# marbl/MashMap

Measured on AMD Instinct MI355X. Metric: query Gbp/s sketch+L1/L2 map (pi=85, s=5000), higher is better.
Workload: dtype u64

## Files before the change

mashmap_amd/csrc/mm_api.hip:

```cpp
#include <chrono>
#include "mm_internal.h"
#include <algorithm>
#include <cstring>
#include <thread>
#include "../host/mm_stats.hpp"
#include "../host/pack2bit.hpp"

static thread_local std::string g_createErr;

static const char* kKernelNames[MM_K_COUNT] = {
  "k_pack2bit", "k_sketch_fast", "k_sketch_hard", "k_seed_lookup", "k_sort_points",
  "k_l1_sweep", "k_l2_sweep", "k_ref_hash", "k_l2_locate", "k_winnow_tiles", "k_l2_select"};

mm_env mm_read_env() {
  mm_env v;
  v.debug = getenv("MM_DEBUG") != nullptr;
  v.timing = getenv("MASHMAP_HIP_TIMING") != nullptr;
  v.sketchStats = getenv("MM_SKETCH_STATS") != nullptr;
  v.l1Literal = getenv("MM_L1_LITERAL") != nullptr;
  if (const char* e = getenv("MM_L2_PRE_LIMIT")) { const int x = atoi(e); if (x >= 0 && x < 4000) v.l2PreLimit = x; }
  if (const char* e = getenv("MM_L2_STREAM_MIB")) { const double x = atof(e); if (x > 0) v.l2StreamMiB = x; }
  v.winnowGsk = getenv("MM_WINNOW_GSK") != nullptr;
  if (const char* e = getenv("MM_SEED_TAGS")) v.seedTags = atoi(e) != 0;
  if (const char* e = getenv("MASHMAP_HIP_RCCL")) v.rcclPath = e;
  v.noRccl = getenv("MASHMAP_HIP_NO_RCCL") != nullptr;
  v.requireRccl = getenv("MASHMAP_HIP_REQUIRE_RCCL") != nullptr;
  return v;
}

std::vector<DevBuf*> mm_ctx::allBufs() {
  DeviceIndex& I = idx;
  return {&I.evKey, &I.evAux, &I.evHash, &I.contigOff, &I.opKey, &I.opAux, &I.opHash, &I.blockOff, &I.evBlock, &I.contigBlock, &I.contigLen, &I.refGroup,
          &I.htSlots, &I.htTags, &I.filter, &I.ptKeys, &I.keys, &I.keyOff, &I.keyFreq, &dMinHits, &dCutoffs, &dAscii, &dAsciiNext, &dReadSrcOff, &dReadPackOff, &dReadLen, &dReadGroup, &dReadSelf, &dReadHasN,
          &dBases2, &dNmask, &dFrags, &dSkHash, &dSkPos, &dSkStrand, &dSkCount, &dHardList, &dCounters, &dSketchSpill, &dSketchTabs, &dQHash, &dQStrand,
          &dStats, &dPtOff, &dPts, &dPtKept, &dPtIds, &dWinFreq, &dWinExt, &dWinHeap, &dWinKeys, &dWinVals, &dWinOffH, &dWinOffT, &dWinCntH, &dWinCntT, &dL1, &dL1b, &dL1Cursors, &dL1Off, &dL1Regions, &dL2, &dL2Info, &dL2Cnt, &dL2Off, &dL2Ops, &dScanTmp, &dL2Tmp, &dL2Wide, &dL2Exact, &dL2Cells,
          &dListB, &dListC, &dBigList, &dMidList, &dL2Sort[0], &dL2Sort[1], &dL2Sort[2], &dL2Sort[3], &dL2Order, &dL2OrderPos, &dL2InitCells, &dL2InitState, &dL2First, &dL2Num, &dAccept, &dMinIsz, &dSelCnt, &dSelOff, &dSelHeap, &dFragTab, &dMappings, &dCommCounts, &dGathered};
}

extern "C" {

int mm_abi_version(void) { return MM_ABI_VERSION; }
const char* mm_kernel_name(int which) { return (which >= 0 && which < MM_K_COUNT) ? kKernelNames[which] : "?"; }

const char* mm_last_error(const mm_ctx* ctx) { return ctx ? ctx->err.c_str() : g_createErr.c_str(); }

int mm_create(mm_ctx** out, int device, const mm_params* p) {
  if (!out || !p) { g_createErr = "mm_create: null argument"; return MM_ERR_ARG; }
  *out = nullptr;
  if (p->kmerSize < 1 || p->kmerSize > 64 || p->sketchSize < 1 || p->segLength < p->kmerSize) {
    g_createErr = "mm_create: unsupported parameters (need 1 <= kmerSize <= 64, sketchSize >= 1, segLength >= kmerSize)";
    return MM_ERR_ARG;
  }
  if (mm_check_params(p, g_createErr) != MM_OK) return MM_ERR_ARG;
  int ndev = 0;
  hipError_t e = hipGetDeviceCount(&ndev);
  if (e != hipSuccess || ndev <= 0 || device < 0 || device >= ndev) {
    g_createErr = std::string("mm_create: no usable HIP device (") + (e == hipSuccess ? "index out of range" : hipGetErrorString(e)) + ")";
    return MM_ERR_DEVICE;
  }
  if ((e = hipSetDevice(device)) != hipSuccess) { g_createErr = hipGetErrorString(e); return MM_ERR_DEVICE; }
  hipDeviceProp_t prop;
  if ((e = hipGetDeviceProperties(&prop, device)) != hipSuccess) { g_createErr = hipGetErrorString(e); return MM_ERR_DEVICE; }
  if (std::string(prop.gcnArchName).find("gfx950") == std::string::npos) {
    g_createErr = std::string("mm_create: kernels are built for gfx950 only, device is ") + prop.gcnArchName;
    return MM_ERR_DEVICE;
  }
  mm_ctx* c = new mm_ctx();
  c->device = device; c->P = *p; c->env = mm_read_env();
  if ((e = hipStreamCreateWithFlags(&c->stream, hipStreamNonBlocking)) != hipSuccess ||
      (e = hipEventCreate(&c->evA)) != hipSuccess || (e = hipEventCreate(&c->evB)) != hipSuccess) {
    g_createErr = hipGetErrorString(e); delete c; return MM_ERR_DEVICE;
  }
  *out = c;
  return MM_OK;
}

void mm_destroy(mm_ctx* c) {
  if (!c) return;
  (void)hipSetDevice(c->device);
  (void)hipStreamSynchronize(c->stream);
  if (c->gatherThread.joinable()) c->gatherThread.join();
  mm_comm_release(c);
  if (c->commStream) (void)hipStreamDestroy(c->commStream);
  if (c->copyStream) { (void)hipStreamSynchronize(c->copyStream); (void)hipStreamDestroy(c->copyStream); }
  if (c->copyDone) (void)hipEventDestroy(c->copyDone);
  for (DevBuf* b : c->allBufs()) b->release();
  c->dGatherSrc.release();
  for (auto& p : c->parked)
    for (DevBuf* b : {&p.dReadSrcOff, &p.dReadPackOff, &p.dReadLen, &p.dReadGroup, &p.dReadSelf, &p.dReadHasN, &p.dBases2, &p.dNmask, &p.dFrags}) b->release();
  if (c->hPass) (void)hipHostFree(c->hPass);
  for (auto& pr : c->evPool) { (void)hipEventDestroy(pr.first); (void)hipEventDestroy(pr.second); }
  if (c->evA) (void)hipEventDestroy(c->evA);
  if (c->evB) (void)hipEventDestroy(c->evB);
  if (c->stream) (void)hipStreamDestroy(c->stream);
  delete c;
}

int mm_synchronize(mm_ctx* c) { MM_HIP(c, hipStreamSynchronize(c->stream)); return MM_OK; }
void* mm_stream(const mm_ctx* c) { return (void*)c->stream; }

int mm_set_option(mm_ctx* c, int option, int value) {
  if (option == MM_OPT_KEEP_POINTS) { c->keepPoints = value != 0; c->keepFiltered = value == 2; c->ptsCap = 0; return MM_OK; }
  if (option == MM_OPT_KEEP_FULL_INDEX) { c->keepFullIndex = value != 0; return MM_OK; }
  if (option == MM_OPT_RESERVE_FRAGMENTS) { c->reserveFrags = value > 0 ? (size_t)value : 0; return MM_OK; }
  c->err = "mm_set_option: unknown option"; return MM_ERR_ARG;
}

int mm_profile_enable(mm_ctx* c, int on) { c->profile = on != 0; return MM_OK; }
int mm_profile_read(mm_ctx* c, double* ms, uint64_t* launches, int reset) {
  if (!c->evPending.empty()) { MM_HIP(c, hipSetDevice(c->device)); MM_HIP(c, hipStreamSynchronize(c->stream)); mm_profile_collect(c); }
  for (int i = 0; i < MM_K_COUNT; i++) { if (ms) ms[i] = c->kMs[i]; if (launches) launches[i] = c->kLaunches[i]; }
  if (reset) for (int i = 0; i < MM_K_COUNT; i++) { c->kMs[i] = 0; c->kLaunches[i] = 0; }
  return MM_OK;
}

int mm_index_upload(mm_ctx* c, const mm_minmer* minmers, size_t nMinmers, const uint64_t* keys, const uint64_t* offsets,
                    size_t nKeys, const mm_interval_point* points, size_t nPoints, const uint64_t* freqSeeds, size_t nFreq,
                    const int32_t* contigLen, const int32_t* refGroup, size_t nContigs) {
  if ((nMinmers && !minmers) || (nKeys && (!keys || !offsets)) || (nPoints && !points) || (nFreq && !freqSeeds) || !contigLen || !nContigs) {
    c->err = "mm_index_upload: null argument"; return MM_ERR_ARG;
  }
  MM_HIP(c, hipSetDevice(c->device));
  c->mirrorMinmers = c->mirrorMap = false;
  c->hMinmers.assign(minmers, minmers + nMinmers);
  c->hKeys.assign(keys, keys + nKeys);
  c->hOffsets.assign(offsets, offsets + nKeys + (nKeys ? 1 : 0));
  if (!nKeys) c->hOffsets.assign(1, 0);
  c->hPoints.assign(points, points + nPoints);
  c->hFreq.assign(freqSeeds, freqSeeds + nFreq);
  std::sort(c->hFreq.begin(), c->hFreq.end());
  if (c->hOffsets.back() != nPoints) { c->err = "mm_index_upload: offsets[nKeys] != nPoints"; return MM_ERR_ARG; }
  c->mapped = false;
  return mm_build_device_index(c, contigLen, refGroup, nContigs);
}

int mm_set_tables(mm_ctx* c, const int32_t* minHits, size_t nMinHits, const int32_t* cutoffs, size_t nCutoffs) {
  if (!minHits || nMinHits < (size_t)c->P.sketchSize + 1 || !cutoffs || nCutoffs < 2) {
    c->err = "mm_set_tables: need sketchSize+1 minHits entries and the sketchCutoffs table"; return MM_ERR_ARG;
  }
  MM_HIP(c, hipSetDevice(c->device));
  MM_HIP(c, c->dMinHits.ensure(nMinHits * 4));
  MM_HIP(c, c->dCutoffs.ensure(nCutoffs * 4));
  MM_HIP(c, hipMemcpyAsync(c->dMinHits.p, minHits, nMinHits * 4, hipMemcpyHostToDevice, c->stream));
  MM_HIP(c, hipMemcpyAsync(c->dCutoffs.p, cutoffs, nCutoffs * 4, hipMemcpyHostToDevice, c->stream));
  MM_HIP(c, hipStreamSynchronize(c->stream));
  c->nMinHits = nMinHits; c->nCutoffs = nCutoffs;
  return MM_OK;
}

int mm_set_tables_default(mm_ctx* c, float pi) {
  const int s = c->P.sketchSize, k = c->P.kmerSize;
  std::vector<int32_t> mh = mmhost::minHitsTable(s, k, pi);
  std::vector<int> cut = mmhost::sketchCutoffs(s, k, mmhost::fixed::ANIDiff, mmhost::fixed::ANIDiffConf, (c->P.flags & MM_FLAG_HG_FILTER) != 0);
  std::vector<int32_t> cut32(cut.begin(), cut.end());
  int rc = mm_set_tables(c, mh.data(), mh.size(), cut32.data(), cut32.size());
  if (rc != MM_OK) return rc;
  std::vector<uint8_t> accept; std::vector<int16_t> minIsz;
  mmhost::replayTables(s, k, pi, mmhost::fixed::ANIDiff, true, std::max(1u, std::thread::hardware_concurrency()), accept, minIsz);
  return mm_set_replay_tables(c, accept.data(), minIsz.data(), (size_t)s + 1);
}

float mm_stat_j2md(float j, int k) { return mmhost::Stat::j2md(j, k); }
float mm_stat_md2j(float d, int k) { return mmhost::Stat::md2j(d, k); }
float mm_stat_md_lower_bound(float d, int s, int k, float ci) { return mmhost::Stat::md_lower_bound(d, s, k, ci); }
int mm_stat_min_hits_relaxed(int s, int k, float pi) { return mmhost::Stat::estimateMinimumHitsRelaxed(s, k, pi, mmhost::fixed::confidence_interval); }
int64_t mm_stat_recommended_sketch_size(int k, float pi, int64_t segLength, uint64_t referenceSize) {
  return mmhost::Stat::recommendedSketchSize(mmhost::fixed::pval_cutoff, mmhost::fixed::confidence_interval, k, 4, pi, segLength, referenceSize);
}
int mm_stat_replay_tables(int sketchSize, int k, float percentageIdentity, float ANIDiff, int keepLowPctId, uint8_t* accept, int16_t* minIsz) {
  if (sketchSize < 1 || !accept || !minIsz) return MM_ERR_ARG;
  std::vector<uint8_t> a; std::vector<int16_t> m;
  mmhost::replayTables(sketchSize, k, percentageIdentity, ANIDiff, keepLowPctId != 0, std::max(1u, std::thread::hardware_concurrency()), a, m);
  std::memcpy(accept, a.data(), a.size()); std::memcpy(minIsz, m.data(), m.size() * 2);
  return MM_OK;
}
int mm_stat_sketch_cutoffs(int sketchSize, int k, int hgFilter, int32_t* out, size_t cap) {
  std::vector<int> cut = mmhost::sketchCutoffs(sketchSize, k, mmhost::fixed::ANIDiff, mmhost::fixed::ANIDiffConf, hgFilter != 0);
  size_t n = std::min(cap, cut.size());
  for (size_t i = 0; i < n; i++) out[i] = cut[i];
  return (int)cut.size();
}

static inline void cut_read(mm_ctx* c, std::vector<DFrag>& dfr, size_t r, int32_t len, int64_t pk, int32_t& maxLen, bool& anyLong) {
  const int k = c->P.kmerSize, L = c->P.segLength;
  const bool split = !(c->P.flags & MM_FLAG_NO_SPLIT);
  if (len < k) return;
  if (!split || len <= L) {
    if (len > L) anyLong = true;
    c->hFrags.push_back(mm_fragment{(int32_t)r, 0, len, 0});
    dfr.push_back(DFrag{pk, len, (int32_t)r});
    maxLen = std::max(maxLen, len);
    return;
  }
  const int nfull = len / L;
  for (int i = 0; i < nfull; i++) {
    c->hFrags.push_back(mm_fragment{(int32_t)r, i * L, L, 0});
    dfr.push_back(DFrag{pk + (int64_t)i * L, L, (int32_t)r});
  }
  if (nfull >= 1 && len % L != 0) {
    c->hFrags.push_back(mm_fragment{(int32_t)r, len - L, L, 0});
    dfr.push_back(DFrag{pk + (int64_t)(len - L), L, (int32_t)r});
  }
  maxLen = std::max(maxLen, L);
}

static int finish_upload(mm_ctx* c, size_t nReads, int64_t pk, const std::vector<int64_t>& srcOff, const std::vector<int64_t>& packOff, const std::vector<int32_t>& rlen,
                         const std::vector<int32_t>& grp, const std::vector<int32_t>& self, const std::vector<uint32_t>* hasN32, const std::vector<DFrag>& dfr, bool packOnDevice) {
  MM_HIP(c, hipMemcpyAsync(c->dReadSrcOff.p, srcOff.data(), (nReads + 1) * 8, hipMemcpyHostToDevice, c->stream));
  MM_HIP(c, hipMemcpyAsync(c->dReadPackOff.p, packOff.data(), (nReads + 1) * 8, hipMemcpyHostToDevice, c->stream));
  if (nReads) {
    MM_HIP(c, hipMemcpyAsync(c->dReadLen.p, rlen.data(), nReads * 4, hipMemcpyHostToDevice, c->stream));
    MM_HIP(c, hipMemcpyAsync(c->dReadGroup.p, grp.data(), nReads * 4, hipMemcpyHostToDevice, c->stream));
    MM_HIP(c, hipMemcpyAsync(c->dReadSelf.p, self.data(), nReads * 4, hipMemcpyHostToDevice, c->stream));
  }
  if (hasN32) MM_HIP(c, hipMemcpyAsync(c->dReadHasN.p, hasN32->data(), nReads * 4 + 4, hipMemcpyHostToDevice, c->stream));
  else MM_HIP(c, hipMemsetAsync(c->dReadHasN.p, 0, nReads * 4 + 4, c->stream));
  MM_HIP(c, hipMemsetAsync((char*)c->dBases2.p + pk / 4, 0, 64, c->stream));
  MM_HIP(c, hipMemsetAsync((char*)c->dNmask.p + pk / 8, 0, 64, c->stream));
  if (!dfr.empty()) MM_HIP(c, hipMemcpyAsync(c->dFrags.p, dfr.data(), dfr.size() * sizeof(DFrag), hipMemcpyHostToDevice, c->stream));
  if (packOnDevice) { const int rc = mm_launch_pack(c); if (rc != MM_OK) return rc; }
  MM_HIP(c, hipStreamSynchronize(c->stream));
  return MM_OK;
}

static int ensure_read_buffers(mm_ctx* c, size_t nReads, int64_t pk, size_t nFrags) {
  if (c->reserveFrags > nFrags) {
    const int64_t pkR = (int64_t)c->reserveFrags * (int64_t)c->P.segLength; pk = pkR > pk ? pkR + pkR / 64 : pk;
    nReads = std::max(nReads, c->reserveFrags); nFrags = c->reserveFrags;
  }
  MM_HIP(c, c->dReadSrcOff.ensure((nReads + 1) * 8)); MM_HIP(c, c->dReadPackOff.ensure((nReads + 1) * 8));
  MM_HIP(c, c->dReadLen.ensure(nReads * 4 + 4)); MM_HIP(c, c->dReadGroup.ensure(nReads * 4 + 4)); MM_HIP(c, c->dReadSelf.ensure(nReads * 4 + 4));
  MM_HIP(c, c->dReadHasN.ensure(nReads * 4 + 4));
  MM_HIP(c, c->dBases2.ensure((size_t)pk / 4 + 64)); MM_HIP(c, c->dNmask.ensure((size_t)pk / 8 + 64));
  MM_HIP(c, c->dFrags.ensure(nFrags * sizeof(DFrag) + 16));
  return MM_OK;
}

static int upload_reads_ascii(mm_ctx* c, const void* ascii, bool onDevice, const int64_t* readOffsets, size_t nReads, const int32_t* readRefGroup,
                              const int32_t* readSelfSeqId, int32_t seqCounterBase) {
  if (!readOffsets) { c->err = "mm_reads_upload: null argument"; return MM_ERR_ARG; }
  std::lock_guard<std::mutex> prefetchLock(c->prefetchMu);
  MM_HIP(c, hipSetDevice(c->device));
  std::vector<int64_t> srcOff(nReads + 1), packOff(nReads + 1);
  std::vector<int32_t> rlen(nReads);
  c->hFrags.clear();
  std::vector<DFrag> dfr;
  dfr.reserve(c->hFrags.capacity() ? c->hFrags.capacity() : nReads * 2 + 16);
  int64_t pk = 0; int32_t maxLen = 0; bool anyLong = false;
  for (size_t r = 0; r < nReads; r++) {
    const int64_t len64 = readOffsets[r + 1] - readOffsets[r];
    if (len64 < 0 || len64 > 0x7fffffff) { c->err = "mm_reads_upload: read length out of range (offset_t is int32, base_types.hpp:21)"; return MM_ERR_ARG; }
    srcOff[r] = readOffsets[r]; packOff[r] = pk; rlen[r] = (int32_t)len64;
    cut_read(c, dfr, r, (int32_t)len64, pk, maxLen, anyLong);
    pk += (len64 + 31) / 32 * 32;
  }
  srcOff[nReads] = readOffsets[nReads]; packOff[nReads] = pk;
  c->nReads = nReads; c->nFrags = dfr.size(); c->nPackedBases = (size_t)pk; c->seqCounterBase = seqCounterBase; c->maxFragLen = maxLen;
  c->sketched = false; c->mapped = false; c->fragTabStale = true; c->gathered = false;
  c->windowed = anyLong;
  const size_t srcBase = (size_t)readOffsets[0];
  const size_t nSrc = (size_t)(readOffsets[nReads] - readOffsets[0]);
  if (nSrc && !ascii) { c->err = "mm_reads_upload: null argument"; return MM_ERR_ARG; }
  for (size_t r = 0; r <= nReads; r++) srcOff[r] -= (int64_t)srcBase;
  const bool prefetched = c->prefetchValid && !onDevice && nSrc && c->prefetchPtr == (const void*)((const char*)ascii + srcBase) && c->prefetchBytes == nSrc;
  c->prefetchValid = false;
  c->staged.clear(); c->stagedBytes = 0;
  if (prefetched) { std::swap(c->dAscii, c->dAsciiNext); MM_HIP(c, hipStreamWaitEvent(c->stream, c->copyDone, 0)); }
  else MM_HIP(c, c->dAscii.ensure(nSrc + 64));
  { const int rc = ensure_read_buffers(c, nReads, pk, dfr.size()); if (rc != MM_OK) return rc; }
  if (nSrc && !prefetched) MM_HIP(c, hipMemcpyAsync(c->dAscii.p, (const char*)ascii + srcBase, nSrc, onDevice ? hipMemcpyDeviceToDevice : hipMemcpyHostToDevice, c->stream));
  std::vector<int32_t> grp(nReads, -1), self(nReads, -1);
  if (readRefGroup) grp.assign(readRefGroup, readRefGroup + nReads);
  if (readSelfSeqId) self.assign(readSelfSeqId, readSelfSeqId + nReads);
  return finish_upload(c, nReads, pk, srcOff, packOff, rlen, grp, self, nullptr, dfr, true);
}

static int upload_packed_parts(mm_ctx* c, const mm_packed_part* parts, size_t nParts, int32_t seqCounterBase) {
  if (nParts && !parts) { c->err = "mm_reads_upload_packed: null argument"; return MM_ERR_ARG; }
  std::lock_guard<std::mutex> prefetchLock(c->prefetchMu);
  MM_HIP(c, hipSetDevice(c->device));
  size_t nReads = 0;
  for (size_t p = 0; p < nParts; p++) {
    if (parts[p].nReads && !parts[p].readLengths) { c->err = "mm_reads_upload_packed: null argument"; return MM_ERR_ARG; }
    nReads += parts[p].nReads;
  }
  if (nReads > 0x7fffffff) { c->err = "mm_reads_upload_packed: more than 2^31 reads in one batch"; return MM_ERR_ARG; }
  std::vector<int64_t> srcOff(nReads + 1, 0), packOff(nReads + 1);
  std::vector<int32_t> rlen(nReads), grp(nReads, -1), self(nReads, -1);
  std::vector<uint32_t> hasN32(nReads + 1, 0u);
  std::vector<int64_t> partBase(nParts + 1, 0);
  c->hFrags.clear();
  std::vector<DFrag> dfr;
  dfr.reserve(c->hFrags.capacity() ? c->hFrags.capacity() : nReads * 2 + 16);
  int64_t pk = 0; int32_t maxLen = 0; bool anyLong = false;
  size_t r = 0;
  for (size_t p = 0; p < nParts; p++) {
    const mm_packed_part& P = parts[p];
    partBase[p] = pk;
    int64_t at = 0;
    for (size_t i = 0; i < P.nReads; i++, r++) {
      const int64_t len64 = (int64_t)P.readLengths[i];
      if (len64 < 0) { c->err = "mm_reads_upload_packed: negative read length"; return MM_ERR_ARG; }
      if (P.readStarts) {
        const int64_t want = P.readStarts[i] - P.readStarts[0];
        if (want < at || (want & 31)) { c->err = "mm_reads_upload_packed: readStarts must be ascending multiples of 32 that leave room for every read"; return MM_ERR_ARG; }
        at = want;
      }
      packOff[r] = pk + at; rlen[r] = (int32_t)len64;
      if (P.readRefGroup) grp[r] = P.readRefGroup[i];
      if (P.readSelfSeqId) self[r] = P.readSelfSeqId[i];
      if (P.readHasN) hasN32[r] = P.readHasN[i] ? 1u : 0u;
      else if (len64) {
        if (!P.nmask) { c->err = "mm_reads_upload_packed: null argument"; return MM_ERR_ARG; }
        const uint32_t* w = P.nmask + at / 32; const size_t nw = ((size_t)len64 + 31) / 32;
        uint32_t any = 0; for (size_t j = 0; j < nw; j++) any |= w[j];
        hasN32[r] = any ? 1u : 0u;
      }
      cut_read(c, dfr, r, (int32_t)len64, pk + at, maxLen, anyLong);
      at += (len64 + 31) / 32 * 32;
    }
    if (at && (!P.bases2 || !P.nmask)) { c->err = "mm_reads_upload_packed: null argument"; return MM_ERR_ARG; }
    pk += at;
  }
  partBase[nParts] = pk; packOff[nReads] = pk;
  c->nReads = nReads; c->nFrags = dfr.size(); c->nPackedBases = (size_t)pk; c->seqCounterBase = seqCounterBase; c->maxFragLen = maxLen;
  c->sketched = false; c->mapped = false; c->fragTabStale = true; c->gathered = false;
  c->windowed = anyLong;
  c->prefetchValid = false;
  { const int rc = ensure_read_buffers(c, nReads, pk, dfr.size()); if (rc != MM_OK) return rc; }
  bool waited = false;
  std::vector<char> used(c->staged.size(), 0);
  for (size_t p = 0; p < nParts; p++) {
    const int64_t n = partBase[p + 1] - partBase[p];
    if (!n) continue;
    char* dB = (char*)c->dBases2.p + partBase[p] / 4; char* dM = (char*)c->dNmask.p + partBase[p] / 8;
    size_t hit = c->staged.size();
    for (size_t q = 0; q < c->staged.size(); q++)
      if (!used[q] && c->staged[q].b2 == (const void*)parts[p].bases2 && c->staged[q].nm == (const void*)parts[p].nmask && c->staged[q].nPacked == (size_t)n) { hit = q; break; }
    if (hit < c->staged.size()) {
      if (!waited) { MM_HIP(c, hipStreamWaitEvent(c->stream, c->copyDone, 0)); waited = true; }
      used[hit] = 1;
      const char* src = (const char*)c->dAsciiNext.p + c->staged[hit].off;
      MM_HIP(c, hipMemcpyAsync(dB, src, (size_t)n / 4, hipMemcpyDeviceToDevice, c->stream));
      MM_HIP(c, hipMemcpyAsync(dM, src + (size_t)n / 4, (size_t)n / 8, hipMemcpyDeviceToDevice, c->stream));
    } else {
      MM_HIP(c, hipMemcpyAsync(dB, parts[p].bases2, (size_t)n / 4, hipMemcpyHostToDevice, c->stream));
      MM_HIP(c, hipMemcpyAsync(dM, parts[p].nmask, (size_t)n / 8, hipMemcpyHostToDevice, c->stream));
    }
  }
  const int rc = finish_upload(c, nReads, pk, srcOff, packOff, rlen, grp, self, &hasN32, dfr, false);
  std::vector<mm_ctx::StagedPart> left;
  for (size_t q = 0; q < c->staged.size(); q++) if (!used[q]) left.push_back(c->staged[q]);
  c->staged.swap(left);
  return rc;
}

int mm_reads_upload(mm_ctx* c, const char* bases, const int64_t* readOffsets, size_t nReads, const int32_t* g, const int32_t* s, int32_t base) {
  return upload_reads_ascii(c, bases, false, readOffsets, nReads, g, s, base);
}
int mm_reads_upload_device(mm_ctx* c, const void* dBases, size_t nBases, const int64_t* readOffsets, size_t nReads, const int32_t* g,
                           const int32_t* s, int32_t base) {
  (void)nBases;
  return upload_reads_ascii(c, dBases, true, readOffsets, nReads, g, s, base);
}
int mm_reads_upload_packed(mm_ctx* c, const uint32_t* bases2, const uint32_t* nmask, const uint8_t* readHasN, const int32_t* readLengths, const int64_t* readStarts,
                           size_t nReads, const int32_t* g, const int32_t* s, int32_t base) {
  static const int32_t none = 0;
  mm_packed_part P{bases2, nmask, readHasN, readLengths ? readLengths : &none, nReads ? readStarts : nullptr, nReads, g, s};
  return upload_packed_parts(c, &P, 1, base);
}
int mm_reads_upload_packed_parts(mm_ctx* c, const mm_packed_part* parts, size_t nParts, int32_t base) { return upload_packed_parts(c, parts, nParts, base); }
size_t mm_pack_read(const char* ascii, size_t len, uint32_t* bases2, uint32_t* nmask) { return mmhost::pack2bit(ascii, len, bases2, nmask); }
size_t mm_pack_read_portable(const char* ascii, size_t len, uint32_t* bases2, uint32_t* nmask) { return mmhost::pack2bit_scalar(ascii, len, bases2, nmask); }

int mm_reads_packed_download(mm_ctx* c, uint32_t* bases2, uint32_t* nmask, uint32_t* readHasN, size_t* nPackedBases) {
  if (nPackedBases) *nPackedBases = c->nPackedBases;
  MM_HIP(c, hipSetDevice(c->device));
  if (bases2 && c->nPackedBases) MM_HIP(c, hipMemcpyAsync(bases2, c->dBases2.p, c->nPackedBases / 4, hipMemcpyDeviceToHost, c->stream));
  if (nmask && c->nPackedBases) MM_HIP(c, hipMemcpyAsync(nmask, c->dNmask.p, c->nPackedBases / 8, hipMemcpyDeviceToHost, c->stream));
  if (readHasN && c->nReads) MM_HIP(c, hipMemcpyAsync(readHasN, c->dReadHasN.p, c->nReads * 4, hipMemcpyDeviceToHost, c->stream));
  MM_HIP(c, hipStreamSynchronize(c->stream));
  return MM_OK;
}

static int prefetch_streams(mm_ctx* c) {
  MM_HIP(c, hipSetDevice(c->device));
  if (!c->copyStream) MM_HIP(c, hipStreamCreateWithFlags(&c->copyStream, hipStreamNonBlocking));
  if (!c->copyDone) MM_HIP(c, hipEventCreateWithFlags(&c->copyDone, hipEventDisableTiming));
  return MM_OK;
}

int mm_reads_prefetch(mm_ctx* c, const char* bases, size_t nBytes) {
  std::lock_guard<std::mutex> prefetchLock(c->prefetchMu);
  c->prefetchValid = false;
  if (!bases || !nBytes) return MM_OK;
  { const int rc = prefetch_streams(c); if (rc != MM_OK) return rc; }
  c->staged.clear(); c->stagedBytes = 0;
  MM_HIP(c, c->dAsciiNext.ensure(nBytes + 64));
  MM_HIP(c, hipMemcpyAsync(c->dAsciiNext.p, bases, nBytes, hipMemcpyHostToDevice, c->copyStream));
  MM_HIP(c, hipEventRecord(c->copyDone, c->copyStream));
  c->prefetchPtr = bases; c->prefetchPtr2 = nullptr; c->prefetchBytes = nBytes; c->prefetchPacked = false; c->prefetchValid = true;
  return MM_OK;
}

static int stage_packed(mm_ctx* c, const uint32_t* bases2, const uint32_t* nmask, size_t nPackedBases, size_t reservePackedBases, int* stagedOut = nullptr) {
  if (stagedOut) *stagedOut = 0;
  if (nPackedBases % 32) { c->err = "mm_reads_prefetch_packed: the packed length of a batch is a multiple of 32 bases"; return MM_ERR_ARG; }
  { const int rc = prefetch_streams(c); if (rc != MM_OK) return rc; }
  c->prefetchValid = false;
  const size_t bytes = nPackedBases / 4 + nPackedBases / 8;
  if (c->staged.empty()) {
    const size_t want = std::max(bytes, reservePackedBases / 4 + reservePackedBases / 8) + 64;
    MM_HIP(c, c->dAsciiNext.ensure(want));
    c->stagedBytes = 0;
  }
  auto fits = [&](size_t off) {
    if (off + bytes + 64 > c->dAsciiNext.bytes) return false;
    for (const auto& q : c->staged) { const size_t qb = q.nPacked / 4 + q.nPacked / 8; if (off < q.off + qb && q.off < off + bytes) return false; }
    return true;
  };
  if (!fits(c->stagedBytes)) {
    if (!fits(0)) return MM_OK;
    c->stagedBytes = 0;
  }
  char* dst = (char*)c->dAsciiNext.p + c->stagedBytes;
  MM_HIP(c, hipMemcpyAsync(dst, bases2, nPackedBases / 4, hipMemcpyHostToDevice, c->copyStream));
  MM_HIP(c, hipMemcpyAsync(dst + nPackedBases / 4, nmask, nPackedBases / 8, hipMemcpyHostToDevice, c->copyStream));
  MM_HIP(c, hipEventRecord(c->copyDone, c->copyStream));
  c->staged.push_back(mm_ctx::StagedPart{bases2, nmask, nPackedBases, c->stagedBytes});
  c->stagedBytes += bytes;
  if (stagedOut) *stagedOut = 1;
  return MM_OK;
}

int mm_reads_prefetch_packed(mm_ctx* c, const uint32_t* bases2, const uint32_t* nmask, size_t nPackedBases) {
  std::lock_guard<std::mutex> prefetchLock(c->prefetchMu);
  c->prefetchValid = false;
  c->staged.clear(); c->stagedBytes = 0;
  if (!bases2 || !nmask || !nPackedBases) return MM_OK;
  return stage_packed(c, bases2, nmask, nPackedBases, nPackedBases);
}

int mm_reads_prefetch_packed_append(mm_ctx* c, const uint32_t* bases2, const uint32_t* nmask, size_t nPackedBases, size_t reservePackedBases, int* staged) {
  std::lock_guard<std::mutex> prefetchLock(c->prefetchMu);
  if (staged) *staged = 0;
  if (!bases2 || !nmask || !nPackedBases) return MM_OK;
  return stage_packed(c, bases2, nmask, nPackedBases, reservePackedBases, staged);
}

int mm_reads_prefetch_reserve(mm_ctx* c, size_t reservePackedBases) {
  std::lock_guard<std::mutex> prefetchLock(c->prefetchMu);
  if (!c->staged.empty() || c->prefetchValid) return MM_OK;
  { const int rc = prefetch_streams(c); if (rc != MM_OK) return rc; }
  MM_HIP(c, c->dAsciiNext.ensure(reservePackedBases / 4 + reservePackedBases / 8 + 64));
  return MM_OK;
}

int mm_reads_prefetch_drop(mm_ctx* c) {
  std::lock_guard<std::mutex> prefetchLock(c->prefetchMu);
  c->prefetchValid = false;
  c->staged.clear(); c->stagedBytes = 0;
  return MM_OK;
}

void* mm_host_alloc(size_t bytes) {
  void* p = nullptr;
  if (hipHostMalloc(&p, bytes ? bytes : 1, hipHostMallocDefault) != hipSuccess) return nullptr;
  return p;
}
void mm_host_free(void* p) { if (p) (void)hipHostFree(p); }

int mm_reads_exchange(mm_ctx* c, int slot) {
  if (slot < 0 || slot >= MM_BATCH_SLOTS) { c->err = "mm_reads_exchange: slot out of range"; return MM_ERR_ARG; }
  std::lock_guard<std::mutex> prefetchLock(c->prefetchMu);
  MM_HIP(c, hipSetDevice(c->device));
  MM_HIP(c, hipStreamSynchronize(c->stream));
  mm_ctx::ParkedReads& p = c->parked[slot];
  std::swap(c->nReads, p.nReads); std::swap(c->nFrags, p.nFrags); std::swap(c->nPackedBases, p.nPackedBases);
  std::swap(c->seqCounterBase, p.seqCounterBase); std::swap(c->maxFragLen, p.maxFragLen); std::swap(c->windowed, p.windowed);
  std::swap(c->dReadSrcOff, p.dReadSrcOff); std::swap(c->dReadPackOff, p.dReadPackOff); std::swap(c->dReadLen, p.dReadLen);
  std::swap(c->dReadGroup, p.dReadGroup); std::swap(c->dReadSelf, p.dReadSelf); std::swap(c->dReadHasN, p.dReadHasN);
  std::swap(c->dBases2, p.dBases2); std::swap(c->dNmask, p.dNmask); std::swap(c->dFrags, p.dFrags);
  c->hFrags.swap(p.hFrags);
  c->sketched = false; c->mapped = false; c->fragTabStale = true; c->gathered = false;
  return MM_OK;
}

size_t mm_num_fragments(const mm_ctx* c) { return c->nFrags; }
int mm_fragments_download(mm_ctx* c, mm_fragment* out) {
  if (c->nFrags) std::memcpy(out, c->hFrags.data(), c->nFrags * sizeof(mm_fragment));
  return MM_OK;
}

int mm_sketch_fragments(mm_ctx* c) {
  MM_HIP(c, hipSetDevice(c->device));
  int rc = mm_launch_sketch(c);
  if (rc != MM_OK) return rc;
  MM_HIP(c, hipStreamSynchronize(c->stream));
  if (c->profile) mm_profile_collect(c);
  c->sketched = true;
  return MM_OK;
}

int mm_sketch_download(mm_ctx* c, mm_minmer* out, uint32_t* counts) {
  if (!c->sketched) { c->err = "mm_sketch_download: no sketches resident"; return MM_ERR_STATE; }
  MM_HIP(c, hipSetDevice(c->device));
  const size_t nF = c->nFrags, s = (size_t)c->P.sketchSize;
  std::vector<uint64_t> h(nF * s); std::vector<int2> p(nF * s); std::vector<int8_t> st(nF * s); std::vector<uint32_t> cnt(nF);
  if (nF) {
    MM_HIP(c, hipMemcpyAsync(h.data(), c->dSkHash.p, nF * s * 8, hipMemcpyDeviceToHost, c->stream));
    MM_HIP(c, hipMemcpyAsync(p.data(), c->dSkPos.p, nF * s * 8, hipMemcpyDeviceToHost, c->stream));
    MM_HIP(c, hipMemcpyAsync(st.data(), c->dSkStrand.p, nF * s, hipMemcpyDeviceToHost, c->stream));
    MM_HIP(c, hipMemcpyAsync(cnt.data(), c->dSkCount.p, nF * 4, hipMemcpyDeviceToHost, c->stream));
    MM_HIP(c, hipStreamSynchronize(c->stream));
  }
  for (size_t f = 0; f < nF; f++) {
    if (counts) counts[f] = cnt[f];
    if (!out) continue;
    for (uint32_t r = 0; r < cnt[f]; r++) {
      const size_t o = f * s + r;
      out[o] = mm_minmer{h[o], p[o].x, p[o].y, c->hFrags[f].readId + c->seqCounterBase, (int16_t)st[o], 0};
    }
  }
  return MM_OK;
}

int mm_map_fragments(mm_ctx* c) {
  if (!c->idx.ready) { c->err = "mm_map_fragments: no index resident (mm_index_upload / mm_index_build first)"; return MM_ERR_STATE; }
  if (!c->nMinHits) { c->err = "mm_map_fragments: mm_set_tables first"; return MM_ERR_STATE; }
  MM_HIP(c, hipSetDevice(c->device));
  const auto t0 = std::chrono::steady_clock::now();
  const double a0 = g_mmAllocSeconds;
  int rc = mm_launch_sketch(c);
  if (rc != MM_OK) return rc;
  c->sketched = true;
  const auto t1 = std::chrono::steady_clock::now();
  rc = mm_launch_map(c);
  if (rc != MM_OK) return rc;
  if (!c->lastSteady) { MM_HIP(c, hipStreamSynchronize(c->stream)); c->nSyncs++; }
  if (c->env.timing && !c->lastSteady) {
    auto sec = [](std::chrono::steady_clock::time_point a, std::chrono::steady_clock::time_point b) { return std::chrono::duration<double>(b - a).count(); };
    fprintf(stderr, "[mashmap_hip::timing] sized pass (%zu fragments, %llu host waits): sketch launch %.4f s, lookup .. selection %.4f s, of both in hipMalloc / hipFree %.4f s\n",
            c->nFrags, (unsigned long long)c->nSyncs, sec(t0, t1), sec(t1, std::chrono::steady_clock::now()), g_mmAllocSeconds - a0);
  }
  if (c->profile) mm_profile_collect(c);
  c->mapped = true;
  c->nPasses++; if (c->lastSteady) c->nSteadyPasses++;
  return MM_OK;
}

int mm_pass_totals(const mm_ctx* c, uint64_t* passes, uint64_t* steadyPasses, uint64_t* redonePasses) {
  if (passes) *passes = c->nPasses;
  if (steadyPasses) *steadyPasses = c->nSteadyPasses;
  if (redonePasses) *redonePasses = c->nRedone;
  return MM_OK;
}

int mm_pass_redo_cause(const mm_ctx* c, uint64_t* cause) {
  if (cause) *cause = c->redoCause;
  return MM_OK;
}

int mm_pass_stats(const mm_ctx* c, uint64_t* hostSyncs, int* steady, uint64_t* counts) {
  if (!c->mapped) return MM_ERR_STATE;
  if (hostSyncs) *hostSyncs = c->nSyncs;
  if (steady) *steady = c->lastSteady ? 1 : 0;
  if (counts) { counts[0] = c->nL1; counts[1] = c->nL2; counts[2] = c->lastBig; counts[3] = c->lastOps; counts[4] = c->lastHard; }
  return MM_OK;
}

int mm_result_counts(const mm_ctx* c, size_t* nL1, size_t* nL2) {
  if (!c->mapped) return MM_ERR_STATE;
  if (nL1) *nL1 = c->nL1;
  if (nL2) *nL2 = c->nL2;
  return MM_OK;
}

int mm_results_device(const mm_ctx* c, const mm_l2_locus** dL2, size_t* nL2) {
  if (!c->mapped) return MM_ERR_STATE;
  if (dL2) *dL2 = c->dL2.as<mm_l2_locus>();
  if (nL2) *nL2 = c->nL2;
  return MM_OK;
}

int mm_results_copy_device(mm_ctx* c, mm_l2_locus* dDst, size_t cap, size_t* n) {
  if (!c->mapped) { c->err = "mm_results_copy_device: nothing mapped"; return MM_ERR_STATE; }
  if (n) *n = c->nL2;
  if (c->nL2 > cap) { c->err = "mm_results_copy_device: destination too small"; return MM_ERR_ARG; }
  if (c->nL2) MM_HIP(c, hipMemcpyAsync(dDst, c->dL2.p, c->nL2 * sizeof(mm_l2_locus), hipMemcpyDeviceToDevice, c->stream));
  MM_HIP(c, hipStreamSynchronize(c->stream));
  return MM_OK;
}

int mm_index_sizes(const mm_ctx* c, size_t* nMinmers, size_t* nKeys, size_t* nPoints, size_t* nFreq, int32_t* freqThreshold) {
  if (!c->idx.ready) return MM_ERR_STATE;
  if (nMinmers) *nMinmers = c->idx.nRec;
  if (nKeys) *nKeys = c->idx.nKeys;
  if (nPoints) *nPoints = c->idx.nPoints;
  if (nFreq) *nFreq = c->hFreq.size();
  if (freqThreshold) *freqThreshold = c->freqThreshold;
  return MM_OK;
}

int mm_index_layout_get(const mm_ctx* c, mm_index_layout* o) {
  if (!c->idx.ready || !o) return MM_ERR_STATE;
  const DeviceIndex& I = c->idx;
  o->seedTableSlots = I.htCap; o->seedTableBytes = (uint64_t)I.htCap * 16;
  o->tagged = I.tagged ? 1 : 0; o->pad_ = 0;
  o->tagBytes = I.tagged ? (uint64_t)I.htCap : 0;
  o->filterBytes = I.filterMask ? (I.filterMask + 1) * 8 : 0;
  o->events = 2 * (uint64_t)I.nRec; o->openRecords = I.nOpen;
  return MM_OK;
}

int mm_index_download(mm_ctx* c, mm_minmer* minmers, uint64_t* keys, uint64_t* offsets, mm_interval_point* points, uint64_t* freqSeeds) {
  if (!c->idx.ready) { c->err = "mm_index_download: no index resident"; return MM_ERR_STATE; }
  if (c->idx.keys.bytes == 0 && c->idx.nKeys) { c->err = "mm_index_download: this context holds a replica (mm_index_replicate); ask the context the index was built on"; return MM_ERR_STATE; }
  MM_HIP(c, hipSetDevice(c->device));
  if (minmers) { const int rc = mm_mirror_minmers(c); if (rc != MM_OK) return rc; }
  if (keys || offsets || points) { const int rc = mm_mirror_map(c); if (rc != MM_OK) return rc; }
  if (minmers && !c->hMinmers.empty()) std::memcpy(minmers, c->hMinmers.data(), c->hMinmers.size() * sizeof(mm_minmer));
  if (keys && !c->hKeys.empty()) std::memcpy(keys, c->hKeys.data(), c->hKeys.size() * 8);
  if (offsets) std::memcpy(offsets, c->hOffsets.data(), c->hOffsets.size() * 8);
  if (points && !c->hPoints.empty()) std::memcpy(points, c->hPoints.data(), c->hPoints.size() * sizeof(mm_interval_point));
  if (freqSeeds && !c->hFreq.empty()) std::memcpy(freqSeeds, c->hFreq.data(), c->hFreq.size() * 8);
  return MM_OK;
}

}
```

mashmap_amd/csrc/mm_internal.h:

```cpp
#pragma once
#include <chrono>
#include <hip/hip_runtime.h>
#include <stdint.h>
#include <mutex>
#include <string>
#include <thread>
#include <utility>
#include <vector>
#include "../../include/mashmap_hip.h"

#define MM_WAVE 64

inline double g_mmAllocSeconds = 0.0;
struct DevBuf {
  void* p = nullptr;
  size_t bytes = 0;
  hipError_t ensure(size_t need) {
    if (need <= bytes) return hipSuccess;
    const auto t0 = std::chrono::steady_clock::now();
    void* q = nullptr;
    size_t cap = need + need / 8 + 256;
    hipError_t e = hipMalloc(&q, cap);
    if (e != hipSuccess) {
      (void)hipGetLastError();
      if (p) { (void)hipFree(p); p = nullptr; bytes = 0; }
      e = hipMalloc(&q, cap);
      if (e != hipSuccess) { (void)hipGetLastError(); cap = need + 256; e = hipMalloc(&q, cap); }
    } else if (p) {
      (void)hipFree(p);
    }
    if (e == hipSuccess) { p = q; bytes = cap; }
    g_mmAllocSeconds += std::chrono::duration<double>(std::chrono::steady_clock::now() - t0).count();
    return e;
  }
  void release() { if (p) (void)hipFree(p); p = nullptr; bytes = 0; }
  template <class T> T* as() const { return reinterpret_cast<T*>(p); }
};

struct DFrag {
  int64_t base;
  int32_t len;
  int32_t readId;
};


#define MM_OPEN_BLOCK_SHIFT 10

struct DeviceIndex {
  size_t nRec = 0, nKeys = 0, nPoints = 0, nContigs = 0, htCap = 0, nOpen = 0;
  DevBuf evKey;
  DevBuf evAux;
  DevBuf evHash;
  DevBuf contigOff;
  DevBuf opKey, opAux, opHash;
  DevBuf blockOff;
  DevBuf evBlock;
  DevBuf contigBlock;
  DevBuf contigLen;
  DevBuf refGroup;
  DevBuf htSlots;
  DevBuf filter; uint64_t filterMask = 0;
  DevBuf htTags; bool tagged = false;
  DevBuf ptKeys;
  DevBuf keys, keyOff, keyFreq;
  bool ready = false;
};

enum : int {
  MM_CW_SKETCH        = 0,
  MM_CW_SKETCH_END    = 8,
  MM_CW_PASS          = 8,
  MM_CW_PASS_END      = 16,
  MM_CW_SORT_LENS     = 16,
  MM_CW_SORT_LENS_END = 18,
  MM_CW_INDEX_BUILD   = 16,
  MM_CW_INDEX_FLATTEN = 20,
  MM_CW_INDEX_END     = 24,
  MM_CW_MID_LEN       = 24,
  MM_CW_SKETCH_PHASES = 24,
  MM_CW_SKETCH_PHASES_END = 32,
  MM_CW_MAP           = 32,
  MM_CW_MAP_END       = 40,
  MM_CW_HARD_COPY     = 48,
  MM_CW_WORDS         = 64
};
#define MM_COUNTER_BYTES ((size_t)MM_CW_WORDS * 8)

enum : int {
  MM_PC_POINT_CURSOR   = 0,
  MM_PC_L2_EXACT_LEN   = 0,
  MM_PC_POINT_OVERFLOW = 1,
  MM_PC_L1_CAND        = 2,
  MM_PC_L1_OVERFLOW    = 3,
  MM_PC_L2_LOCI        = 4,
  MM_PC_L2_OVERFLOW    = 5,
  MM_PC_L2_FLAGS       = 6,
  MM_PC_BIG_LEN        = 7,
  MM_PC_L2_WIDE_LEN    = 7,
  MM_PC_READ           = MM_CW_PASS_END - MM_CW_PASS,
  MM_PC_MID_LEN        = MM_CW_MID_LEN - MM_CW_PASS
};
constexpr unsigned long long MM_OVERFLOWED = 1ull;
constexpr unsigned long long MM_L2F_SLOTS  = 1ull;
constexpr unsigned long long MM_L2F_STREAM = 4ull;
constexpr unsigned long long MM_L2F_OPS    = 8ull;
constexpr unsigned long long MM_L2F_LIST   = 16ull;
constexpr unsigned long long MM_L2F_CANDS  = 32ull;
__host__ __device__ inline bool mm_pass_incomplete(const unsigned long long* pc) {
  return (pc[MM_PC_POINT_OVERFLOW] | pc[MM_PC_L1_OVERFLOW] | pc[MM_PC_L2_OVERFLOW] | pc[MM_PC_L2_FLAGS]) != 0;
}
enum : int {
  MM_MC_MAPPINGS = 0,
  MM_MC_OVERFLOW = 1,
  MM_MC_L2_OPS   = 2
};
inline uint64_t mm_redo_cause(const unsigned long long* pc, const unsigned long long* mc) {
  const unsigned long long f = pc[MM_PC_L2_FLAGS];
  uint64_t cause = 0;
  if (pc[MM_PC_POINT_OVERFLOW]) cause |= MM_REDO_POINTS;
  if (pc[MM_PC_L1_OVERFLOW]) cause |= MM_REDO_L1;
  if (pc[MM_PC_L2_OVERFLOW]) cause |= MM_REDO_L2_LOCI;
  if (f & MM_L2F_SLOTS) cause |= MM_REDO_L2_SLOTS;
  if (f & MM_L2F_STREAM) cause |= MM_REDO_L2_STREAM;
  if (f & MM_L2F_OPS) cause |= MM_REDO_L2_OPS;
  if (f & MM_L2F_LIST) cause |= MM_REDO_L2_LIST;
  if (f & MM_L2F_CANDS) cause |= MM_REDO_L2_CANDS;
  if (mc[MM_MC_OVERFLOW]) cause |= MM_REDO_MAPPINGS;
  return cause;
}
enum : int {
  MM_SL_BLOCK   = 0,
  MM_SL_GLOBAL  = 1,
  MM_SL_LITERAL = 2,
  MM_SL_END     = 4
};
enum : int {
  MM_IX_BUILD_UNSTABLE = 0,
  MM_IX_BUILD_NFREQ    = 1,
  MM_IX_BUILD_CURSOR   = 2,
  MM_IX_BUILD_THRESHOLD = 3,
  MM_IX_FLAT_BAD_REC   = 1,
  MM_IX_FLAT_MAX_LEN   = 2,
  MM_IX_FLAT_TABLE     = 3
};
static_assert(MM_CW_SKETCH_END <= MM_CW_PASS && MM_CW_PASS_END <= MM_CW_SORT_LENS && MM_CW_SORT_LENS_END <= MM_CW_MID_LEN, "mapping pass: parts overlap");
static_assert(MM_CW_SORT_LENS * 2 + MM_SL_END <= MM_CW_SORT_LENS_END * 2, "the 32-bit list lengths outgrow their words");
static_assert(MM_CW_MID_LEN < MM_CW_MAP && MM_CW_MAP + MM_MC_L2_OPS < MM_CW_MAP_END && MM_CW_MAP_END <= MM_CW_HARD_COPY && MM_CW_HARD_COPY < MM_CW_WORDS, "mapping pass: parts overlap");
static_assert(MM_CW_INDEX_BUILD + 4 == MM_CW_INDEX_FLATTEN && MM_CW_INDEX_FLATTEN + 4 == MM_CW_INDEX_END && MM_CW_SKETCH_END <= MM_CW_INDEX_BUILD, "index build: parts overlap");
static_assert(MM_CW_SKETCH_PHASES >= MM_CW_INDEX_END && MM_CW_SKETCH_PHASES_END <= MM_CW_MAP, "the sketch statistics must stay clear of the words that outlive the sketch launcher");
static_assert(MM_PC_POINT_CURSOR == MM_PC_L2_EXACT_LEN && MM_PC_BIG_LEN == MM_PC_L2_WIDE_LEN, "the words shared by the L1 stage and the L2 sweep");
static_assert(MM_CW_PASS + MM_PC_MID_LEN == MM_CW_SKETCH_PHASES, "k_lookup_mid's list length shares its word with the sketch statistics");
static_assert(MM_PC_L2_LOCI + 1 == MM_PC_L2_OVERFLOW && MM_PC_L2_OVERFLOW + 1 == MM_PC_L2_FLAGS && MM_PC_L2_FLAGS < MM_PC_READ, "the L2 words are reset as one range");
static_assert(MM_PC_L1_CAND + 1 == MM_PC_L1_OVERFLOW, "the L1 cursor and its flag are read back as one range");

struct mm_env {
  bool debug = false;
  bool timing = false;
  bool sketchStats = false;
  bool l1Literal = false;
  int l2PreLimit = 4000;
  double l2StreamMiB = 0;
  bool winnowGsk = false;
  int seedTags = -1;
  std::string rcclPath;
  bool noRccl = false;
  bool requireRccl = false;
};
mm_env mm_read_env();

struct mm_ctx {
  int device = 0;
  hipStream_t stream = nullptr;
  mm_params P{};
  mm_env env;
  std::string err;

  std::vector<mm_minmer> hMinmers;
  std::vector<mm_minmer> hMinmersAll;
  bool keepFullIndex = false;
  std::vector<uint64_t> hKeys, hOffsets, hFreq;
  std::vector<mm_interval_point> hPoints;
  bool mirrorMinmers = false, mirrorMap = false;
  int32_t freqThreshold = 0x7fffffff;

  DeviceIndex idx;
  DevBuf dMinHits, dCutoffs; size_t nMinHits = 0, nCutoffs = 0;

  size_t nReads = 0, nFrags = 0, nPackedBases = 0;
  int32_t seqCounterBase = 0, maxFragLen = 0;
  DevBuf dAscii, dReadSrcOff, dReadPackOff, dReadLen, dReadGroup, dReadSelf, dReadHasN;
  DevBuf dAsciiNext; hipStream_t copyStream = nullptr; hipEvent_t copyDone = nullptr;
  const void* prefetchPtr = nullptr; const void* prefetchPtr2 = nullptr; size_t prefetchBytes = 0; bool prefetchValid = false, prefetchPacked = false;
  struct StagedPart { const void* b2; const void* nm; size_t nPacked; size_t off; };
  std::vector<StagedPart> staged; size_t stagedBytes = 0;
  std::mutex prefetchMu;
  DevBuf dBases2, dNmask, dFrags;
  std::vector<mm_fragment> hFrags;
  struct ParkedReads {
    size_t nReads = 0, nFrags = 0, nPackedBases = 0; int32_t seqCounterBase = 0, maxFragLen = 0; bool windowed = false;
    DevBuf dReadSrcOff, dReadPackOff, dReadLen, dReadGroup, dReadSelf, dReadHasN, dBases2, dNmask, dFrags;
    std::vector<mm_fragment> hFrags;
  };
  ParkedReads parked[MM_BATCH_SLOTS];

  DevBuf dSkHash, dSkPos, dSkStrand, dSkCount;
  DevBuf dHardList, dCounters, dSketchSpill;
  DevBuf dSketchTabs; int sketchTabsK = 0;
  DevBuf dQHash, dQStrand;
  DevBuf dStats;
  DevBuf dPtOff, dPts; size_t ptsCap = 0;
  DevBuf dPtKept;
  bool windowed = false;
  DevBuf dPtIds, dWinFreq, dWinExt, dWinHeap, dWinKeys, dWinVals, dWinOffH, dWinOffT, dWinCntH, dWinCntT;
  DevBuf dL1, dL1b, dL1Cursors; size_t l1Cap = 0, nL1 = 0;
  DevBuf dL1Off;
  DevBuf dL1Regions;
  DevBuf dL2; size_t l2Cap = 0, nL2 = 0;
  DevBuf dL2First, dL2Num;
  DevBuf dAccept, dMinIsz; bool haveReplayTables = false;
  DevBuf dSelCnt, dSelOff, dSelHeap, dFragTab, dMappings; size_t nMappings = 0; bool fragTabStale = true;
  void* comm = nullptr; int commRank = 0, commWorld = 0; bool commCopy = false;
  DevBuf dCommCounts, dGathered; std::vector<size_t> gatherCounts, gatherDisp; size_t nGathered = 0; bool gathered = false;
  DevBuf dGatherSrc; hipStream_t commStream = nullptr; std::thread gatherThread; int gatherRc = 0; std::string gatherErr;
  std::vector<DevBuf*> allBufs();
  DevBuf dL2Info, dL2Cnt, dL2Off, dL2Ops, dScanTmp, dL2Tmp, dL2Wide, dL2Exact, dL2Cells, dListB, dListC, dBigList, dMidList;
  DevBuf dL2InitCells, dL2InitState;
  DevBuf dL2Sort[4], dL2Order, dL2OrderPos;
  bool sketched = false, mapped = false;
  bool steadyOk = false, lastSteady = false; size_t prevBig = 0, candCap = 0, l2Chunks = 1, sizedFrags = 0; int prevLocap = 0, steadyFails = 0;
  unsigned long long* hPass = nullptr;
  size_t lastHard = 0;
  size_t prevMid = 0, lastMid = 0; bool midKnown = false;
  size_t lastOps = 0, lastBig = 0;
  size_t nSyncs = 0;
  uint64_t nPasses = 0, nSteadyPasses = 0, nRedone = 0;
  uint64_t redoCause = 0;
  bool keepFiltered = false;
  bool keepPoints = false;
  size_t reserveFrags = 0;

  bool profile = false;
  double kMs[MM_K_COUNT] = {0};
  uint64_t kLaunches[MM_K_COUNT] = {0};
  hipEvent_t evA = nullptr, evB = nullptr;
  std::vector<std::pair<hipEvent_t, hipEvent_t>> evPool; size_t evUsed = 0;
  std::vector<std::pair<int, size_t>> evPending;
};

#define MM_HIP(ctx, call)                                                                        \
  do {                                                                                           \
    hipError_t e__ = (call);                                                                     \
    if (e__ != hipSuccess) {                                                                     \
      (ctx)->err = std::string(#call) + ": " + hipGetErrorString(e__);                           \
      return MM_ERR_DEVICE;                                                                      \
    }                                                                                            \
  } while (0)
#define MM_SYNC(c) do { MM_HIP(c, hipStreamSynchronize((c)->stream)); (c)->nSyncs++; } while (0)

struct KernelTimer {
  mm_ctx* c; int which; size_t idx = 0; bool on = false;
  KernelTimer(mm_ctx* c_, int w) : c(c_), which(w) {
    if (!c->profile) return;
    if (c->evUsed == c->evPool.size()) {
      if (c->evPool.size() >= 8192) return;
      hipEvent_t a = nullptr, b = nullptr;
      if (hipEventCreate(&a) != hipSuccess || hipEventCreate(&b) != hipSuccess) { if (a) (void)hipEventDestroy(a); c->profile = false; return; }
      c->evPool.emplace_back(a, b);
    }
    idx = c->evUsed++;
    on = hipEventRecord(c->evPool[idx].first, c->stream) == hipSuccess;
  }
  ~KernelTimer() {
    if (!on) return;
    if (hipEventRecord(c->evPool[idx].second, c->stream) == hipSuccess) c->evPending.emplace_back(which, idx);
  }
};
inline void mm_profile_collect(mm_ctx* c) {
  for (const auto& pr : c->evPending) {
    float ms = 0;
    if (hipEventElapsedTime(&ms, c->evPool[pr.second].first, c->evPool[pr.second].second) == hipSuccess) { c->kMs[pr.first] += ms; c->kLaunches[pr.first] += 1; }
  }
  c->evPending.clear(); c->evUsed = 0;
}

inline size_t mm_frag_cap(const mm_ctx* c, size_t nF) { return nF > c->reserveFrags ? nF : c->reserveFrags; }
inline size_t mm_scaled(const mm_ctx* c, size_t count, size_t bytesPer) {
  const size_t nF = c->nFrags ? c->nFrags : 1;
  if (c->reserveFrags <= nF) return count;
  size_t scaled = (size_t)((double)count * (double)c->reserveFrags / (double)nF) + 1;
  size_t freeB = 0, totalB = 0;
  if (hipMemGetInfo(&freeB, &totalB) != hipSuccess) { (void)hipGetLastError(); return count; }
  const size_t most = freeB / 8 / (bytesPer ? bytesPer : 1);
  if (scaled > most) scaled = most > count ? most : count;
  return scaled;
}

int mm_check_params(const mm_params* p, std::string& err);
int mm_launch_pack(mm_ctx* c);
int mm_launch_pack_raw(mm_ctx* c, const uint8_t* dAscii, const int64_t* dSrcOff, const int64_t* dPackOff, const int32_t* dLen, int nReads,
                       int64_t nChunks, uint32_t* dB, uint32_t* dM, uint32_t* dHasN);
int mm_launch_sketch(mm_ctx* c);
int mm_launch_sketch_global(mm_ctx* c);
#define MM_LDS_MAX_SKETCH 8190
#define MM_WINNOW_LDS_SKETCH 4096
#define MM_MAX_SKETCH 65535
int mm_launch_map(mm_ctx* c);
#define MM_PASS_REDO 1
int mm_launch_select(mm_ctx* c, bool steady = false);
void mm_comm_release(mm_ctx* c);
int mm_launch_l2(mm_ctx* c, unsigned long long* cnt, bool steady = false);
int mm_build_device_index(mm_ctx* c, const int32_t* contigLen, const int32_t* refGroup, size_t nContigs);
int mm_flatten_device_index(mm_ctx* c, const mm_minmer* dRec, size_t n, size_t nk, size_t np, const int32_t* contigLen, const int32_t* refGroup, size_t nContigs);
int mm_finalize_index_device(mm_ctx* c, const std::vector<std::pair<const mm_minmer*, size_t>>& parts, float kmerPctThreshold, const int32_t* contigLen,
                             const int32_t* refGroup, size_t nContigs);
int mm_mirror_minmers(mm_ctx* c);
int mm_mirror_map(mm_ctx* c);
int mm_scan_i32_to_i64(mm_ctx* c, int64_t n, const int32_t* dIn, int64_t* dOut, int64_t* total);
int mm_scan_i32_to_i64_dev(mm_ctx* c, int64_t n, const int32_t* dIn, int64_t* dOut, const int64_t** dTotal);
int mm_order_desc(mm_ctx* c, const int32_t* dKey, int c0, int n, int shift, int32_t* dOrder);
int mm_order_pairs(mm_ctx* c, int n, unsigned bits, int32_t* dOrder);
```

mashmap_amd/csrc/mm_sketch.hip:

```cpp
#include "mm_internal.h"
#include "mm_device.h"
#include <cmath>
#include <cstdio>
#include <cstdlib>

__global__ void k_pack2bit(const uint8_t* __restrict__ ascii, const int64_t* __restrict__ srcOff,
                           const int64_t* __restrict__ packOff, const int32_t* __restrict__ readLen, int nReads,
                           int64_t nChunks, uint32_t* __restrict__ bases2, uint32_t* __restrict__ nmask,
                           uint32_t* __restrict__ readHasN) {
  for (int64_t c = (int64_t)blockIdx.x * blockDim.x + threadIdx.x; c < nChunks; c += (int64_t)gridDim.x * blockDim.x) {
    const int64_t b0 = c * 32;
    int lo = 0, hi = nReads;
    while (hi - lo > 1) { int mid = (lo + hi) >> 1; if (packOff[mid] <= b0) lo = mid; else hi = mid; }
    const int r = lo;
    const int64_t local = b0 - packOff[r];
    const int len = readLen[r];
    uint32_t wlo = 0, whi = 0, nm = 0;
    if (local < len) {
      const uint8_t* src = ascii + srcOff[r] + local;
      const int cnt = (len - local) < 32 ? (int)(len - local) : 32;
      for (int i = 0; i < cnt; i++) {
        const uint32_t ch = src[i] & 0xDFu;
        const bool ok = (ch == 'A') | (ch == 'C') | (ch == 'G') | (ch == 'T');
        const uint32_t code = ok ? (((ch >> 1) ^ (ch >> 2)) & 3u) : 0u;
        if (i < 16) wlo |= code << (2 * i); else whi |= code << (2 * (i - 16));
        nm |= (ok ? 0u : 1u) << i;
      }
    }
    bases2[2 * c] = wlo; bases2[2 * c + 1] = whi;
    nmask[c] = nm;
    if (nm) atomicOr(&readHasN[r], 1u);
  }
}

#define MM_SK_PAD 64
#define MM_SK_PADH 256
#define MM_SK_DUPCAP 256
#define MM_SK_GUARD 4
enum : int { MM_TC_KEYS = 0 , MM_TC_OVERFLOW = 1 , MM_TC_OCCUPIED = 2 , MM_TC_DUPS = 3  };
struct SkTable {
  uint64_t* key; int32_t* first; int32_t* last; int32_t* sum;
  uint32_t* counters;
  uint64_t* occW; uint32_t* occP;
  uint32_t nSlots, maxLoad, M; int sh;

  __device__ __forceinline__ void set_cut(uint64_t T, uint32_t HT) {
    sh = (T == MM_HASH_MAX) ? 0 : __clzll((long long)T);
    const uint64_t t32 = ((T << sh) >> 32) + 1ull;
    M = (uint32_t)((float)HT * 4294967296.0f / (float)t32 * 0.99999f);
  }
  __device__ __forceinline__ uint32_t home(uint64_t h) const { return __umulhi((uint32_t)((h << sh) >> 32), M); }

  __device__ __forceinline__ void insert(uint64_t h, int pos, int st) {
    uint32_t slot = home(h);
    for (uint32_t probes = 1;; probes++) {
      if ((probes & 15u) == 0 && ((volatile uint32_t*)counters)[MM_TC_OVERFLOW]) return;
      const unsigned long long prev = atomicCAS((unsigned long long*)&key[slot], (unsigned long long)MM_HASH_MAX,
                                                (unsigned long long)h);
      if (prev == MM_HASH_MAX) {
        if (atomicAdd(&counters[MM_TC_KEYS], 1u) >= maxLoad) atomicOr(&counters[MM_TC_OVERFLOW], 1u);
      }
      if (prev == MM_HASH_MAX || prev == h) {
        atomicMin(&first[slot], pos); atomicMax(&last[slot], pos); atomicAdd(&sum[slot], st);
        return;
      }
      if (++slot >= nSlots) { atomicOr(&counters[MM_TC_OVERFLOW], 1u); return; }
    }
  }
};

__host__ __device__ static inline int sketch_fast_queue_total(int QC, int nWaves, int HT) { const int a = QC * nWaves, b = HT * 5 / 8 + 1; return ((a > b ? a : b) + 3) & ~3; }

template <int K>
__device__ __forceinline__ uint64_t mm_window_or(uint64_t x) {
  constexpr int P = K >= 32 ? 32 : K >= 16 ? 16 : K >= 8 ? 8 : K >= 4 ? 4 : K >= 2 ? 2 : 1;
  uint64_t w = x;
#pragma unroll
  for (int d = 1; d < P; d <<= 1) w |= w >> d;
  return w | (w >> (K - P));
}

#define MM_SK_HINT_OVERFLOW 0xFFFFFFFFu
template <int K, bool SPILL>
__device__ __forceinline__ void
mm_sketch_hard(unsigned char* smem, const int f, const uint4* __restrict__ gTabs, const uint32_t* __restrict__ bases2, const uint32_t* __restrict__ nmask,
               const DFrag* __restrict__ frags, const uint32_t* __restrict__ readHasN, int s, int wantFast, int HT, int PAD, int32_t* __restrict__ spill,
               const bool stream ,
               uint64_t* __restrict__ skHash, int2* __restrict__ skPos, int8_t* __restrict__ skStrand, uint32_t* __restrict__ skCount) {
  const DFrag fr = frags[f];
  const int len = fr.len;
  const int n = len - K + 1;
  const int tid = threadIdx.x, nthr = blockDim.x;
  if (n <= 0) { if (tid == 0) skCount[f] = 0; return; }
  const bool hasN = readHasN[fr.readId] != 0;
  const uint32_t hint = skCount[f];

  const int nW = stream ? 0 : (len + 15) / 16 + 3;
  const int nM = stream ? 0 : (len + 31) / 32 + 2;
  const int NS = HT + PAD;
  const int nOcc = NS >> 6;
  size_t off = 0;
  using Tabs = typename MMTabsFor<K>::type;
  Tabs* tabs = (Tabs*)(smem + off); off += sizeof(Tabs);
  static_assert(sizeof(Tabs) % 16 == 0, "tables are copied in 16-byte pieces");
  for (int i = tid; i < (int)(sizeof(Tabs) / 16); i += nthr) ((uint4*)tabs)[i] = gTabs[i];
  uint32_t* sW = (uint32_t*)(smem + off); off += (((size_t)nW * 4 + 15) / 16) * 16;
  uint32_t* sM = (uint32_t*)(smem + off); off += (((size_t)nM * 4 + 15) / 16) * 16;
  SkTable tab;
  tab.key = (uint64_t*)(smem + off) + MM_SK_GUARD; off += (size_t)(NS + 2 * MM_SK_GUARD) * 8;
  tab.occW = (uint64_t*)(smem + off); off += (size_t)nOcc * 8;
  if constexpr (SPILL) {
    int32_t* g = spill + (size_t)blockIdx.x * 3 * (size_t)NS;
    tab.first = g; tab.last = g + NS; tab.sum = g + 2 * (size_t)NS;
  } else {
    tab.first = (int32_t*)(smem + off); off += (size_t)NS * 4;
    tab.last = (int32_t*)(smem + off); off += (size_t)NS * 4;
    tab.sum = (int32_t*)(smem + off); off += (size_t)NS * 4;
  }
  tab.occP = (uint32_t*)(smem + off); off += (((size_t)nOcc * 4 + 15) / 16) * 16;
  tab.counters = (uint32_t*)(smem + off); off += 16;
  tab.nSlots = (uint32_t)NS; tab.maxLoad = (uint32_t)HT * 5u / 8u;

  const int64_t gw0 = fr.base >> 4; const int gsh = (int)(fr.base & 15) * 2;
  const int64_t gm0 = fr.base >> 5; const int gmsh = (int)(fr.base & 31);
  {
    for (int j = tid; j < nW; j += nthr) {
      const uint32_t a = bases2[gw0 + j], b = bases2[gw0 + j + 1];
      sW[j] = gsh ? __builtin_amdgcn_alignbit(b, a, gsh) : a;
    }
    if (hasN) {
      for (int j = tid; j < nM; j += nthr) {
        const uint32_t a = nmask[gm0 + j], b = nmask[gm0 + j + 1];
        sM[j] = gmsh ? __builtin_amdgcn_alignbit(b, a, gmsh) : a;
      }
    }
  }
  auto wordAt = [&](int j) -> uint32_t {
    if (!stream) return sW[j];
    const uint32_t a = bases2[gw0 + j], b = bases2[gw0 + j + 1];
    return gsh ? __builtin_amdgcn_alignbit(b, a, gsh) : a;
  };
  auto maskAt = [&](int j) -> uint32_t {
    if (!stream) return sM[j];
    const uint32_t a = nmask[gm0 + j], b = nmask[gm0 + j + 1];
    return gmsh ? __builtin_amdgcn_alignbit(b, a, gmsh) : a;
  };

  auto scaled = [&](uint64_t T, uint32_t D) -> uint64_t {
    float r = 1.6f * (float)s / (float)(D ? D : 1u);
    if (r < 2.0f) r = 2.0f;
    const float t = (float)T * r;
    return t >= 1.8e19f ? MM_HASH_MAX : (uint64_t)t;
  };
  uint64_t T = ((uint32_t)wantFast >= (uint32_t)n) ? MM_HASH_MAX : (uint64_t)((float)wantFast / (float)(2 * n) * 18446744073709551616.0f);
  if (hint != MM_SK_HINT_OVERFLOW && T != MM_HASH_MAX) T = scaled(T, hint);
  uint64_t lo = 0, hi = MM_HASH_MAX; bool hiInf = true;
  const int nStrips = (n + 15) >> 4;
  uint32_t D = 0;

  for (int attempt = 0;; attempt++) {
    tab.set_cut(T, (uint32_t)HT);
    for (int i = tid; i < NS; i += nthr) { tab.key[i] = MM_HASH_MAX; tab.first[i] = 0x7fffffff; tab.last[i] = -1; tab.sum[i] = 0; }
    if (tid < MM_SK_GUARD) { tab.key[-1 - tid] = MM_HASH_MAX; tab.key[NS + tid] = MM_HASH_MAX; }
    if (tid < 4) tab.counters[tid] = 0;
    if constexpr (SPILL) __threadfence();
    __syncthreads();

    const bool allPass = (T == MM_HASH_MAX);
    for (int strip = tid; strip < nStrips; strip += nthr) {
      const int rem = n - strip * 16;
      uint32_t ok = rem >= 16 ? 0xFFFFu : ((1u << rem) - 1u);
      if (hasN) {
        const uint64_t m64 = (uint64_t)maskAt(strip >> 1) | ((uint64_t)maskAt((strip >> 1) + 1) << 32);
        if constexpr (MMWideK<K>::value) {
          const uint64_t h64 = (uint64_t)maskAt((strip >> 1) + 2) | ((uint64_t)maskAt((strip >> 1) + 3) << 32);
          const int sh = (strip & 1) * 16;
          ok &= ~mm_window_or_wide<K>(sh ? ((m64 >> sh) | (h64 << (64 - sh))) : m64, sh ? (h64 >> sh) : h64);
        } else ok &= ~(uint32_t)mm_window_or<K>(m64 >> ((strip & 1) * 16));
      }
      auto onPos = [&](int j, uint64_t hf, uint64_t hr) {
        const int pos = strip * 16 + j;
        const uint64_t h = hf < hr ? hf : hr;
        bool pass = false;
        if ((ok & (1u << j)) != 0) { if (hf != hr) { if (allPass || h < T) pass = true; } }
        if (pass) tab.insert(h, pos, hf < hr ? 1 : -1);
      };
      if constexpr (MMWideK<K>::value) {
        uint32_t ww[MMWideK<K>::NW];
#pragma unroll
        for (int i = 0; i < MMWideK<K>::NW; i++) ww[i] = wordAt(strip + i);
        mm_strip_hashes_wide<K>(ww, *tabs, onPos);
      } else mm_strip_hashes<K>(wordAt(strip), wordAt(strip + 1), wordAt(strip + 2), *tabs, onPos);
    }
    if constexpr (SPILL) __threadfence();
    __syncthreads();

    for (int base = 0; base < NS; base += nthr) {
      const int slot = base + tid;
      if (slot < NS) {
        const uint64_t m = __ballot(tab.key[slot] != MM_HASH_MAX);
        if (mm_lane() == 0) tab.occW[slot >> 6] = m;
      }
    }
    __syncthreads();
    if (tid < 64) {
      int carry = 0;
      for (int w0 = 0; w0 < nOcc; w0 += 64) {
        const int w = w0 + tid;
        const int v = w < nOcc ? (int)__popcll(tab.occW[w]) : 0;
        const int ex = mm_wave_excl_scan(v);
        if (w < nOcc) tab.occP[w] = (uint32_t)(carry + ex);
        carry += mm_wave_sum(v);
      }
      if (tid == 0) tab.counters[MM_TC_OCCUPIED] = (uint32_t)carry;
    }
    __syncthreads();

    D = tab.counters[MM_TC_OCCUPIED];
    const bool overflow = tab.counters[MM_TC_OVERFLOW] != 0;
    if (overflow) { hi = T; hiInf = false; }
    else if (D < (uint32_t)s && T != MM_HASH_MAX) { lo = T; }
    else break;
    T = hiInf ? scaled(T, D) : lo + (hi - lo) / 2;
    __syncthreads();
    if (attempt > 200) break;
  }

  for (int slot = tid; slot < NS; slot += nthr) {
    const uint64_t k = tab.key[slot];
    if (k == MM_HASH_MAX) continue;
    uint64_t L[MM_SK_GUARD], Rr[MM_SK_GUARD];
#pragma unroll
    for (int i = 0; i < MM_SK_GUARD; i++) { L[i] = tab.key[slot - 1 - i]; Rr[i] = tab.key[slot + 1 + i]; }
    uint32_t smaller = 0;
    int q = slot;
    bool openL = true, openR = true;
#pragma unroll
    for (int i = 0; i < MM_SK_GUARD; i++) {
      openL = openL && L[i] != MM_HASH_MAX;
      openR = openR && Rr[i] != MM_HASH_MAX;
      if (openL) { smaller += L[i] < k ? 1u : 0u; q = slot - 1 - i; }
      if (openR) smaller += Rr[i] < k ? 1u : 0u;
    }
    if (openL) { while (q > 0) { const uint64_t o = tab.key[q - 1]; if (o == MM_HASH_MAX) break; smaller += o < k ? 1u : 0u; q--; } }
    if (openR) { for (int r = slot + 1 + MM_SK_GUARD; r < NS; r++) { const uint64_t o = tab.key[r]; if (o == MM_HASH_MAX) break; smaller += o < k ? 1u : 0u; } }
    const uint64_t below = tab.occW[q >> 6] & ((1ull << (q & 63)) - 1ull);
    const uint32_t rank = tab.occP[q >> 6] + (uint32_t)__popcll(below) + smaller;
    if (rank < (uint32_t)s) {
      const size_t o = (size_t)f * s + rank;
      skHash[o] = k;
      int vf, vl, vs;
      if constexpr (SPILL) {
        vf = __hip_atomic_load(&tab.first[slot], __ATOMIC_RELAXED, __HIP_MEMORY_SCOPE_AGENT);
        vl = __hip_atomic_load(&tab.last[slot], __ATOMIC_RELAXED, __HIP_MEMORY_SCOPE_AGENT);
        vs = __hip_atomic_load(&tab.sum[slot], __ATOMIC_RELAXED, __HIP_MEMORY_SCOPE_AGENT);
      } else { vf = tab.first[slot]; vl = tab.last[slot]; vs = tab.sum[slot]; }
      skPos[o] = make_int2(vf, vl);
      const int16_t acc = (int16_t)vs;
      skStrand[o] = acc > 0 ? 1 : (acc == 0 ? 0 : -1);
    }
  }
  if (tid == 0) skCount[f] = D < (uint32_t)s ? D : (uint32_t)s;
}

template <int K, bool SPILL>
__global__ void __launch_bounds__(1024)
k_sketch_hard(const uint4* __restrict__ gTabs, const uint32_t* __restrict__ bases2, const uint32_t* __restrict__ nmask,
              const DFrag* __restrict__ frags, const uint32_t* __restrict__ readHasN,
              const int32_t* __restrict__ fragList, const uint32_t* __restrict__ fragListCount, int s, int wantFast, int HT, int PAD, int32_t* __restrict__ spill, int stream,
              uint64_t* __restrict__ skHash, int2* __restrict__ skPos, int8_t* __restrict__ skStrand, uint32_t* __restrict__ skCount) {
  extern __shared__ __attribute__((aligned(16))) unsigned char smem[];
  const uint32_t nList = *fragListCount;
  for (uint32_t i = blockIdx.x; i < nList; i += gridDim.x) {
    mm_sketch_hard<K, SPILL>(smem, fragList[i], gTabs, bases2, nmask, frags, readHasN, s, wantFast, HT, PAD, spill, stream != 0, skHash, skPos, skStrand, skCount);
    __syncthreads();
  }
}

__global__ void __launch_bounds__(256)
k_sketch_all_hard(int nF, int32_t* __restrict__ hardList, uint32_t* __restrict__ hardCount, uint32_t* __restrict__ skCount) {
  const int f = blockIdx.x * 256 + threadIdx.x;
  if (f < nF) { hardList[f] = f; skCount[f] = MM_SK_HINT_OVERFLOW; }
  if (f == 0) *hardCount = (uint32_t)nF;
}

#define MM_SKF_FLAG 0x80000000u
struct SkFast {
  uint64_t* key; uint32_t* meta;
  uint32_t* dup; uint32_t* counters;
  uint64_t* occW; uint32_t* occP;
  uint32_t nSlots, maxLoad, M; int sh;
  __device__ __forceinline__ void set_cut(uint64_t T, uint32_t HT) {
    sh = (T == MM_HASH_MAX) ? 0 : __clzll((long long)T);
    const uint64_t t32 = ((T << sh) >> 32) + 1ull;
    M = (uint32_t)((float)HT * 4294967296.0f / (float)t32 * 0.99999f);
  }
  __device__ __forceinline__ uint32_t home(uint64_t h) const { return __umulhi((uint32_t)((h << sh) >> 32), M); }
  __device__ __forceinline__ void insert(uint64_t h, uint32_t m) {
    uint32_t slot = home(h);
    for (;;) {
      const unsigned long long prev = atomicCAS((unsigned long long*)&key[slot], (unsigned long long)MM_HASH_MAX, (unsigned long long)h);
      if (prev == MM_HASH_MAX) { meta[slot] = m; return; }
      if (prev == h) {
        const uint32_t at = atomicAdd(&counters[MM_TC_DUPS], 1u);
        if (at < MM_SK_DUPCAP) dup[at] = slot | (m << 13); else atomicOr(&counters[MM_TC_OVERFLOW], 1u);
        return;
      }
      if (++slot >= nSlots) { atomicOr(&counters[MM_TC_OVERFLOW], 1u); return; }
    }
  }
};

template <int K, int SL>
__device__ __forceinline__ void
mm_sketch_fast(unsigned char* smem, const int f, const uint4* __restrict__ gTabs, const uint32_t* __restrict__ bases2, const uint32_t* __restrict__ nmask,
               const DFrag* __restrict__ frags, const uint32_t* __restrict__ readHasN, int s, int wantFast, int HT, int PAD, int QC,
               uint64_t* __restrict__ skHash, int2* __restrict__ skPos, int8_t* __restrict__ skStrand,
               uint32_t* __restrict__ skCount, int32_t* __restrict__ hardList, uint32_t* __restrict__ hardCount,
               unsigned long long* __restrict__ phaseStats) {
  unsigned long long tPrev = phaseStats ? __builtin_amdgcn_s_memtime() : 0ull;
  auto mark = [&](int ph) {
    if (phaseStats && threadIdx.x == 0) { const unsigned long long t = __builtin_amdgcn_s_memtime(); atomicAdd(&phaseStats[ph], t - tPrev); tPrev = t; }
  };
  const DFrag fr = frags[f];
  const int len = fr.len;
  const int n = len - K + 1;
  const int tid = threadIdx.x, nthr = blockDim.x;
  if (n <= 0) { if (tid == 0) skCount[f] = 0; return; }
  const bool hasN = readHasN[fr.readId] != 0;

  const int nW = (len + 15) / 16 + 4;
  const int nM = (len + 31) / 32 + 3;
  const int NS = HT + PAD;
  const int nOcc = NS >> 6;
  const int nWaves = nthr >> 6;
  const int QTOT = sketch_fast_queue_total(QC, nWaves, HT);
  size_t off = 0;
  using Tabs = typename MMTabsFor<K>::type;
  Tabs* tabs = (Tabs*)(smem + off); off += sizeof(Tabs);
  for (int i = tid; i < (int)(sizeof(Tabs) / 16); i += nthr) ((uint4*)tabs)[i] = gTabs[i];
  uint32_t* sW = (uint32_t*)(smem + off); off += (((size_t)nW * 4 + 15) / 16) * 16;
  uint32_t* sM = (uint32_t*)(smem + off); off += (((size_t)nM * 4 + 15) / 16) * 16;
  uint64_t* qH = (uint64_t*)(smem + off); off += (size_t)QC * nWaves * 8;
  uint32_t* qM = (uint32_t*)(smem + off); off += (size_t)QTOT * 4;
  SkFast tab;
  tab.key = (uint64_t*)(smem + off) + MM_SK_GUARD; off += (size_t)(NS + 2 * MM_SK_GUARD) * 8;
  tab.occW = (uint64_t*)(smem + off); off += (size_t)nOcc * 8;
  tab.meta = (uint32_t*)(smem + off); off += (size_t)NS * 4;
  tab.occP = (uint32_t*)(smem + off); off += (((size_t)nOcc * 4 + 15) / 16) * 16;
  uint32_t* qCnt = (uint32_t*)(smem + off); off += 64;
  tab.dup = (uint32_t*)(smem + off); off += (size_t)MM_SK_DUPCAP * 4;
  tab.counters = (uint32_t*)(smem + off); off += 16;
  tab.nSlots = (uint32_t)NS; tab.maxLoad = (uint32_t)HT * 5u / 8u;

  {
    const int64_t w0 = fr.base >> 4; const int sh = (int)(fr.base & 15) * 2;
    for (int j = tid; j < nW; j += nthr) {
      const uint32_t a = bases2[w0 + j], b = bases2[w0 + j + 1];
      sW[j] = sh ? __builtin_amdgcn_alignbit(b, a, sh) : a;
    }
    if (hasN) {
      const int64_t m0 = fr.base >> 5; const int msh = (int)(fr.base & 31);
      for (int j = tid; j < nM; j += nthr) {
        const uint32_t a = nmask[m0 + j], b = nmask[m0 + j + 1];
        sM[j] = msh ? __builtin_amdgcn_alignbit(b, a, msh) : a;
      }
    }
  }
  const uint64_t T = ((uint32_t)wantFast >= (uint32_t)n) ? MM_HASH_MAX : (uint64_t)((float)wantFast / (float)(2 * n) * 18446744073709551616.0f);
  const int nStrips = (n + SL - 1) / SL;
  tab.set_cut(T, (uint32_t)HT);
  for (int i = tid; i < NS; i += nthr) tab.key[i] = MM_HASH_MAX;
  if (tid < MM_SK_GUARD) { tab.key[-1 - tid] = MM_HASH_MAX; tab.key[NS + tid] = MM_HASH_MAX; }
  if (tid < 4) tab.counters[tid] = 0;
  __syncthreads();
  mark(0);

  const uint32_t qBase = (uint32_t)(tid >> 6) * (uint32_t)QC, qEnd = qBase + (uint32_t)QC;
  uint32_t qHead = qBase;
  const uint64_t allPassM = (T == MM_HASH_MAX) ? ~0ull : 0ull;
  for (int strip = tid; strip < nStrips; strip += nthr) {
    const int b0 = strip * SL;
    const int wi = b0 >> 4, bsh = (b0 & 15) * 2;
    const int rem = n - b0;
    uint32_t ok = rem >= SL ? (uint32_t)((1ull << SL) - 1ull) : ((1u << rem) - 1u);
    if (hasN) {
      const int mi = b0 >> 5, msh = b0 & 31;
      const uint64_t lo64 = (uint64_t)sM[mi] | ((uint64_t)sM[mi + 1] << 32);
      if constexpr (MMWideK<K>::value) {
        const uint64_t hi64 = (uint64_t)sM[mi + 2] | ((uint64_t)sM[mi + 3] << 32);
        const uint64_t lo = msh ? ((lo64 >> msh) | (hi64 << (64 - msh))) : lo64, hi = msh ? (hi64 >> msh) : hi64;
        ok &= ~mm_window_or_wide<K>(lo, hi);
      } else {
        const uint64_t m64 = msh ? ((lo64 >> msh) | ((uint64_t)sM[mi + 2] << (64 - msh))) : lo64;
        ok &= ~(uint32_t)mm_window_or<K>(m64);
      }
    }
    auto onPos = [&](int j, uint64_t hf, uint64_t hr) {
      const int pos = b0 + j;
      const uint64_t mLt = mm_mask_lt64(hf, hr);
      const uint64_t h = mm_mask_select64(mLt, hf, hr);
      const uint64_t m = mm_mask_nz32(ok & (1u << j)) & mm_mask_ne64(hf, hr) & (mm_mask_lt64(h, T) | allPassM);
      const uint32_t idx = __builtin_amdgcn_mbcnt_hi((uint32_t)(m >> 32), __builtin_amdgcn_mbcnt_lo((uint32_t)m, qHead));
      if (__builtin_amdgcn_inverse_ballot_w64(m) && idx < qEnd) { qH[idx] = h; qM[idx] = ((uint32_t)pos << 1) | (__builtin_amdgcn_inverse_ballot_w64(mLt) ? 1u : 0u); }
      qHead += (uint32_t)__popcll(m);
    };
    if constexpr (MMWideK<K>::value) {
      uint32_t ww[MMWideK<K>::NW];
#pragma unroll
      for (int i = 0; i < MMWideK<K>::NW; i++) ww[i] = sW[wi + i];
      mm_strip_hashes_wide<K>(ww, *tabs, onPos);
    } else {
      uint32_t w0 = sW[wi], w1 = sW[wi + 1], w2 = sW[wi + 2];
      if (SL % 16 != 0) {
        const uint32_t w3 = sW[wi + 3];
        if (bsh) { w0 = __builtin_amdgcn_alignbit(w1, w0, bsh); w1 = __builtin_amdgcn_alignbit(w2, w1, bsh); w2 = __builtin_amdgcn_alignbit(w3, w2, bsh); }
      }
      mm_strip_hashes<K, SL>(w0, w1, w2, *tabs, onPos);
    }
  }
  mark(1);
  {
    const uint32_t qCount = (uint32_t)__builtin_amdgcn_readfirstlane((int)(qHead - qBase));
    if (mm_lane() == 0) { qCnt[tid >> 6] = qCount; if (qCount > (uint32_t)QC) atomicOr(&tab.counters[MM_TC_OVERFLOW], 1u); }
  }
  __syncthreads();
  mark(2);
  if (tab.counters[MM_TC_OVERFLOW] == 0) {
    uint32_t pre[17]; pre[0] = 0;
#pragma unroll
    for (int w = 0; w < 16; w++) pre[w + 1] = pre[w] + (w < nWaves ? qCnt[w] : 0u);
    const uint32_t total = pre[16];
    if (nWaves <= 4) {
      const uint32_t p1 = pre[1], p2 = pre[2], p3 = pre[3];
      for (uint32_t g = (uint32_t)tid; g < total; g += (uint32_t)nthr) {
        const uint32_t w = (g >= p1 ? 1u : 0u) + (g >= p2 ? 1u : 0u) + (g >= p3 ? 1u : 0u);
        const uint32_t start = g >= p3 ? p3 : (g >= p2 ? p2 : (g >= p1 ? p1 : 0u));
        const uint32_t at = w * (uint32_t)QC + (g - start);
        tab.insert(qH[at], qM[at]);
      }
    } else
    for (uint32_t g = (uint32_t)tid; g < total; g += (uint32_t)nthr) {
      uint32_t w = 0, start = 0;
#pragma unroll
      for (int x = 1; x < 16; x++) if (g >= pre[x]) { w = (uint32_t)x; start = pre[x]; }
      const uint32_t at = w * (uint32_t)QC + (g - start);
      tab.insert(qH[at], qM[at]);
    }
  }
  __syncthreads();
  mark(3);
  {
    const uint32_t nd = tab.counters[MM_TC_DUPS] < MM_SK_DUPCAP ? tab.counters[MM_TC_DUPS] : MM_SK_DUPCAP;
    for (uint32_t i = (uint32_t)tid; i < nd; i += (uint32_t)nthr) atomicOr(&tab.meta[tab.dup[i] & 0x1FFFu], MM_SKF_FLAG);
  }
  for (int base = 0; base < NS; base += nthr) {
    const int slot = base + tid;
    if (slot < NS) {
      const uint64_t m = __ballot(tab.key[slot] != MM_HASH_MAX);
      if (mm_lane() == 0) tab.occW[slot >> 6] = m;
    }
  }
  __syncthreads();
  if (tid < 64) {
    int carry = 0;
    for (int w0 = 0; w0 < nOcc; w0 += 64) {
      const int w = w0 + tid;
      const int v = w < nOcc ? (int)__popcll(tab.occW[w]) : 0;
      const int ex = mm_wave_excl_scan(v);
      if (w < nOcc) tab.occP[w] = (uint32_t)(carry + ex);
      carry += mm_wave_sum(v);
    }
    if (tid == 0) { tab.counters[MM_TC_OCCUPIED] = (uint32_t)carry; if ((uint32_t)carry > tab.maxLoad) tab.counters[MM_TC_OVERFLOW] = 1u; }
  }
  __syncthreads();
  const uint32_t D = tab.counters[MM_TC_OCCUPIED];
  if (tab.counters[MM_TC_OVERFLOW] != 0 || (D < (uint32_t)s && T != MM_HASH_MAX)) {
    if (tid == 0) { const uint32_t at = atomicAdd(hardCount, 1u); hardList[at] = f; skCount[f] = tab.counters[MM_TC_OVERFLOW] != 0 ? MM_SK_HINT_OVERFLOW : D; }
    return;
  }
  uint32_t* occList = qM;
  for (int slot = tid; slot < NS; slot += nthr) {
    const uint64_t m = tab.occW[slot >> 6];
    if ((m >> (slot & 63)) & 1ull) occList[tab.occP[slot >> 6] + (uint32_t)__popcll(m & ((1ull << (slot & 63)) - 1ull))] = (uint32_t)slot;
  }
  __syncthreads();
  mark(4);

  const uint32_t nDup = tab.counters[MM_TC_DUPS];
  for (int it = tid; it < (int)D; it += nthr) {
    const int slot = (int)occList[it];
    const uint64_t k = tab.key[slot];
    uint64_t L[MM_SK_GUARD], Rr[MM_SK_GUARD];
#pragma unroll
    for (int i = 0; i < MM_SK_GUARD; i++) { L[i] = tab.key[slot - 1 - i]; Rr[i] = tab.key[slot + 1 + i]; }
    uint32_t smaller = 0;
    int q = slot;
    bool openL = true, openR = true;
#pragma unroll
    for (int i = 0; i < MM_SK_GUARD; i++) {
      openL = openL && L[i] != MM_HASH_MAX;
      openR = openR && Rr[i] != MM_HASH_MAX;
      if (openL) { smaller += L[i] < k ? 1u : 0u; q = slot - 1 - i; }
      if (openR) smaller += Rr[i] < k ? 1u : 0u;
    }
    if (openL) { while (q > 0) { const uint64_t o = tab.key[q - 1]; if (o == MM_HASH_MAX) break; smaller += o < k ? 1u : 0u; q--; } }
    if (openR) { for (int r = slot + 1 + MM_SK_GUARD; r < NS; r++) { const uint64_t o = tab.key[r]; if (o == MM_HASH_MAX) break; smaller += o < k ? 1u : 0u; } }
    const uint32_t rank = (uint32_t)(it - (slot - q)) + smaller;
    if (rank < (uint32_t)s) {
      const uint32_t m = tab.meta[slot];
      int first = (int)((m & ~MM_SKF_FLAG) >> 1), last = first, sum = (m & 1u) ? 1 : -1;
      if (m & MM_SKF_FLAG) {
        for (uint32_t i = 0; i < nDup; i++) {
          const uint32_t d = tab.dup[i];
          if ((int)(d & 0x1FFFu) != slot) continue;
          const int pos = (int)(d >> 14);
          first = pos < first ? pos : first; last = pos > last ? pos : last; sum += ((d >> 13) & 1u) ? 1 : -1;
        }
      }
      const size_t o = (size_t)f * s + rank;
      skHash[o] = k;
      skPos[o] = make_int2(first, last);
      const int16_t acc = (int16_t)sum;
      skStrand[o] = acc > 0 ? 1 : (acc == 0 ? 0 : -1);
    }
  }
  if (tid == 0) skCount[f] = D < (uint32_t)s ? D : (uint32_t)s;
  mark(5);
}

template <int K, int SL>
__global__ void __launch_bounds__(1024)
k_sketch_fast(const uint4* __restrict__ gTabs, const uint32_t* __restrict__ bases2, const uint32_t* __restrict__ nmask,
              const DFrag* __restrict__ frags, const uint32_t* __restrict__ readHasN, int s, int wantFast, int HT, int PAD, int QC,
              uint64_t* __restrict__ skHash, int2* __restrict__ skPos, int8_t* __restrict__ skStrand,
              uint32_t* __restrict__ skCount, int32_t* __restrict__ hardList, uint32_t* __restrict__ hardCount,
              unsigned long long* __restrict__ phaseStats) {
  extern __shared__ __attribute__((aligned(16))) unsigned char smem[];
  mm_sketch_fast<K, SL>(smem, (int)blockIdx.x, gTabs, bases2, nmask, frags, readHasN, s, wantFast, HT, PAD, QC, skHash, skPos, skStrand, skCount,
                        hardList, hardCount, phaseStats);
}

template <int K, int SL>
__global__ void __launch_bounds__(1024)
k_hash_only(const uint4* __restrict__ gTabs, const uint32_t* __restrict__ bases2, const DFrag* __restrict__ frags, uint64_t* __restrict__ sink) {
  extern __shared__ __attribute__((aligned(16))) unsigned char smem[];
  const DFrag fr = frags[blockIdx.x];
  const int len = fr.len, n = len - K + 1;
  const int tid = threadIdx.x, nthr = blockDim.x;
  if (n <= 0) return;
  using Tabs = typename MMTabsFor<K>::type;
  Tabs* tabs = (Tabs*)smem;
  for (int i = tid; i < (int)(sizeof(Tabs) / 16); i += nthr) ((uint4*)tabs)[i] = gTabs[i];
  uint32_t* sW = (uint32_t*)(smem + sizeof(Tabs));
  const int nW = (len + 15) / 16 + 4;
  {
    const int64_t w0 = fr.base >> 4; const int sh = (int)(fr.base & 15) * 2;
    for (int j = tid; j < nW; j += nthr) {
      const uint32_t a = bases2[w0 + j], b = bases2[w0 + j + 1];
      sW[j] = sh ? __builtin_amdgcn_alignbit(b, a, sh) : a;
    }
  }
  __syncthreads();
  const int nStrips = (n + SL - 1) / SL;
  uint64_t acc = 0;
  for (int strip = tid; strip < nStrips; strip += nthr) {
    const int b0 = strip * SL;
    const int wi = b0 >> 4, bsh = (b0 & 15) * 2;
    uint32_t w0 = sW[wi], w1 = sW[wi + 1], w2 = sW[wi + 2];
    if (SL % 16 != 0) {
      const uint32_t w3 = sW[wi + 3];
      if (bsh) { w0 = __builtin_amdgcn_alignbit(w1, w0, bsh); w1 = __builtin_amdgcn_alignbit(w2, w1, bsh); w2 = __builtin_amdgcn_alignbit(w3, w2, bsh); }
    }
    mm_strip_hashes<K, SL>(w0, w1, w2, *tabs, [&](int j, uint64_t hf, uint64_t hr) { acc += hf < hr ? hf : hr; });
  }
  if (acc == 0x9E3779B97F4A7C15ull) sink[0] = acc;
}

template <int K>
__global__ void k_sketch_tables(typename MMTabsFor<K>::type* out) { mm_tables_init<K>(*out, (int)threadIdx.x, (int)blockDim.x); }

static size_t sketch_hard_lds(size_t tabBytes, int maxLen, int HT, int PAD) {
  const size_t nW = (size_t)(maxLen + 15) / 16 + 3, nM = (size_t)(maxLen + 31) / 32 + 2;
  const size_t NS = (size_t)HT + PAD, nOcc = NS / 64;
  return tabBytes + ((nW * 4 + 15) / 16) * 16 + ((nM * 4 + 15) / 16) * 16 + NS * (8 + 4 + 4 + 4) + 2 * MM_SK_GUARD * 8 + nOcc * 8 +
         ((nOcc * 4 + 15) / 16) * 16 + 16;
}
static int next_pow2(int x) { int p = 1; while (p < x) p <<= 1; return p; }

struct FastGeom { int SL, threads, HT, QC, wantFast; size_t lds; };
static size_t sketch_fast_lds(size_t tabBytes, int maxLen, int HT, int PAD, int QC, int nWaves) {
  const size_t nW = (size_t)(maxLen + 15) / 16 + 4, nM = (size_t)(maxLen + 31) / 32 + 3;
  const size_t NS = (size_t)HT + PAD, nOcc = NS / 64;
  return tabBytes + ((nW * 4 + 15) / 16) * 16 + ((nM * 4 + 15) / 16) * 16 + (size_t)QC * nWaves * 8 + (size_t)sketch_fast_queue_total(QC, nWaves, HT) * 4 +
         (NS + 2 * MM_SK_GUARD) * 8 + nOcc * 8 + NS * 4 + ((nOcc * 4 + 15) / 16) * 16 + 64 + (size_t)MM_SK_DUPCAP * 4 + 16;
}
static FastGeom sketch_fast_geom(int K, int s, int maxLen, size_t tabBytes, bool sl20Built) {
  FastGeom g;
  g.wantFast = (int)(s + 4.2 * sqrt((double)s) + 0.999);
  int n = maxLen - K + 1; if (n < 1) n = 1;
  auto wavesFor = [&](int SL) { int st = (n + SL - 1) / SL; int w = (st + 63) / 64; return w < 1 ? 1 : (w > 16 ? 16 : w); };
  g.SL = 16;
  if (sl20Built && 20 + K - 1 <= 48) {
    const int w16 = wavesFor(16), w20 = wavesFor(20);
    const int c16 = ((w16 + 3) / 4) * 16, c20 = ((w20 + 3) / 4) * 20;
    if (c20 < c16 || (c20 == c16 && w20 < w16)) g.SL = 20;
  }
  g.threads = wavesFor(g.SL) * 64;
  const int nWaves = g.threads / 64;
  int nStrips = (n + g.SL - 1) / g.SL; if (nStrips < 1) nStrips = 1;
  const int passes = (nStrips + g.threads - 1) / g.threads;
  double ex = 64.0 * passes * g.SL * (double)g.wantFast / (double)n; if (ex > g.wantFast) ex = g.wantFast;
  auto shape = [&](double htf, double qsig) {
    int HT = (int)(htf * g.wantFast + 63) / 64 * 64; if (HT < 256) HT = 256;
    g.HT = HT;
    g.QC = ((int)(ex + qsig * sqrt(ex) + 8.0) + 3) & ~3;
    g.lds = sketch_fast_lds(tabBytes, maxLen, g.HT, MM_SK_PAD, g.QC, nWaves);
    const size_t unit = 1280, alloc = (g.lds + unit - 1) / unit * unit;
    return (int)((size_t)160 * 1024 / alloc);
  };
  const double cand[3][2] = {{2.4, 6.0}, {2.2, 6.0}, {2.2, 5.0}};
  int best = 0, bestWg = shape(cand[0][0], cand[0][1]);
  for (int i = 1; i < 3; i++) { const int wg = shape(cand[i][0], cand[i][1]); if (wg > bestWg) { bestWg = wg; best = i; } }
  (void)shape(cand[best][0], cand[best][1]);
  return g;
}
static int sketch_ht_hard(int s) { const int w = (s * 16 + 4) / 5; return next_pow2(w < 1024 ? 1024 : w); }

struct SketchPlan { bool ok, useFast, spill, stream = false; FastGeom g; int HTH; size_t ldsFast, ldsHard; };
static size_t sketch_hard_lds_spill(size_t tabBytes, int maxLen, int HT, int PAD) {
  const size_t nW = (size_t)(maxLen + 15) / 16 + 3, nM = (size_t)(maxLen + 31) / 32 + 2;
  const size_t NS = (size_t)HT + PAD, nOcc = NS / 64;
  return tabBytes + ((nW * 4 + 15) / 16) * 16 + ((nM * 4 + 15) / 16) * 16 + NS * 8 + 2 * MM_SK_GUARD * 8 + nOcc * 8 + ((nOcc * 4 + 15) / 16) * 16 + 16;
}
static SketchPlan sketch_plan(int K, int s, int maxLen, size_t tabBytes, bool sl20Built) {
  const size_t lim = 160 * 1024;
  SketchPlan P;
  P.g = sketch_fast_geom(K, s, maxLen, tabBytes, sl20Built);
  P.ldsFast = P.g.lds;
  P.useFast = P.ldsFast <= lim && P.g.HT + MM_SK_PAD <= 8192 && maxLen < (1 << 18);
  P.HTH = sketch_ht_hard(s);
  P.ldsHard = sketch_hard_lds(tabBytes, maxLen, P.HTH, MM_SK_PADH);
  P.spill = P.ldsHard > lim;
  if (P.spill) {
    P.ldsHard = sketch_hard_lds_spill(tabBytes, maxLen, P.HTH, MM_SK_PADH);
    if (P.ldsHard > lim) {
      P.HTH = (((s * 16 + 4) / 5) + 63) / 64 * 64;
      P.ldsHard = sketch_hard_lds_spill(tabBytes, maxLen, P.HTH, MM_SK_PADH);
    }
  }
  if (P.ldsHard > lim) {
    P.stream = true;
    P.HTH = sketch_ht_hard(s);
    P.ldsHard = sketch_hard_lds_spill(tabBytes, 0, P.HTH, MM_SK_PADH);
    if (P.ldsHard > lim) { P.HTH = (((s * 16 + 4) / 5) + 63) / 64 * 64; P.ldsHard = sketch_hard_lds_spill(tabBytes, 0, P.HTH, MM_SK_PADH); }
  }
  P.ok = P.ldsHard <= lim;
  return P;
}

int mm_check_params(const mm_params* p, std::string& err) {
  const int s = p->sketchSize, L = p->segLength;
  const size_t tabBytes = (p->kmerSize >= 16 && p->kmerSize <= 32) ? sizeof(MMProdTables) : sizeof(MMTables);
  const SketchPlan P = sketch_plan(p->kmerSize, s, L, tabBytes, false);
  const size_t lim = 160 * 1024;
  const size_t ldsL2 = (size_t)(s + 1) * 8 * 2;
  int NB = 256; while (NB < s) NB <<= 1;
  const size_t ldsLoc = (size_t)(s + 1) * 8 + (size_t)(s + 2) / 2 * 8 + (size_t)(NB + 4) * 2 + (size_t)s + 32 + (size_t)(s + 4) / 2 * 4 + 16;
  if (s > MM_LDS_MAX_SKETCH) {
    if (s > MM_MAX_SKETCH) {
      err = "mm_create: sketchSize " + std::to_string(s) + " is beyond " + std::to_string(MM_MAX_SKETCH) + " (seeds are numbered in 16 bits by the literal mapping kernels)";
      return MM_ERR_ARG;
    }
    return MM_OK;
  }
  if (!P.ok || ldsL2 > lim || ldsLoc > lim) {
    char b[400];
    snprintf(b, sizeof b, "mm_create: segLength %d with sketchSize %d needs %zu bytes of LDS in the sketch kernel (table of the exact path, spilled form), %zu in the L2 "
             "sweep and %zu in the L2 locate kernel; a CU has %zu (sketchSize up to ~5000)",
             L, s, P.ldsHard, ldsL2, ldsLoc, lim);
    err = b; return MM_ERR_ARG;
  }
  return MM_OK;
}

template <int K> struct MMHasSL20 { static constexpr bool value = (K >= 16 && K <= 21); };

template <int K>
static int launch_sketch_k(mm_ctx* c) {
  const int s = c->P.sketchSize;
  const int nF = (int)c->nFrags;
  using Tabs = typename MMTabsFor<K>::type;
  const int maxLen = c->maxFragLen;
  const SketchPlan plan = sketch_plan(K, s, maxLen, sizeof(Tabs), MMHasSL20<K>::value);
  const FastGeom g = plan.g;
  const int HTH = plan.HTH;
  const int PAD = MM_SK_PAD, PADH = MM_SK_PADH;
  const size_t ldsFast = plan.ldsFast, ldsHard = plan.ldsHard;
  if (!plan.ok) { c->err = "fragment too long / sketch too large for the LDS-resident sketch kernel"; return MM_ERR_ARG; }
  int nStrips = (maxLen - K + 1 + 15) / 16; if (nStrips < 1) nStrips = 1;
  int threadsHard = ((nStrips + 63) / 64) * 64; if (threadsHard > 1024) threadsHard = 1024;
  if (c->sketchTabsK != K) {
    MM_HIP(c, c->dSketchTabs.ensure(sizeof(Tabs)));
    hipLaunchKernelGGL((k_sketch_tables<K>), dim3(1), dim3(256), 0, c->stream, c->dSketchTabs.as<Tabs>());
    MM_HIP(c, hipGetLastError());
    c->sketchTabsK = K;
  }
  MM_HIP(c, hipMemsetAsync(c->dCounters.as<unsigned long long>() + MM_CW_SKETCH, 0, (size_t)(MM_CW_SKETCH_END - MM_CW_SKETCH) * 8, c->stream));
  unsigned long long* phaseStats = nullptr;
  if (c->env.sketchStats) { phaseStats = c->dCounters.as<unsigned long long>() + MM_CW_SKETCH_PHASES; MM_HIP(c, hipMemsetAsync(phaseStats, 0, (size_t)(MM_CW_SKETCH_PHASES_END - MM_CW_SKETCH_PHASES) * 8, c->stream)); }
  if (plan.useFast) {
    KernelTimer t(c, MM_K_SKETCH);
    auto launch = [&](auto kern) {
      (void)hipFuncSetAttribute((const void*)kern, hipFuncAttributeMaxDynamicSharedMemorySize, (int)ldsFast);
      hipLaunchKernelGGL(kern, dim3(nF), dim3(g.threads), ldsFast, c->stream,
                         c->dSketchTabs.as<uint4>(), c->dBases2.as<uint32_t>(), c->dNmask.as<uint32_t>(), c->dFrags.as<DFrag>(), c->dReadHasN.as<uint32_t>(),
                         s, g.wantFast, g.HT, PAD, g.QC, c->dSkHash.as<uint64_t>(), c->dSkPos.as<int2>(), c->dSkStrand.as<int8_t>(),
                         c->dSkCount.as<uint32_t>(), c->dHardList.as<int32_t>(), c->dCounters.as<uint32_t>(), phaseStats);
    };
    if constexpr (MMHasSL20<K>::value) { if (g.SL == 20) launch(k_sketch_fast<K, 20>); else launch(k_sketch_fast<K, 16>); }
    else launch(k_sketch_fast<K, 16>);
    MM_HIP(c, hipGetLastError());
  } else {
    KernelTimer t(c, MM_K_SKETCH);
    hipLaunchKernelGGL(k_sketch_all_hard, dim3((nF + 255) / 256), dim3(256), 0, c->stream, nF, c->dHardList.as<int32_t>(), c->dCounters.as<uint32_t>(), c->dSkCount.as<uint32_t>());
    MM_HIP(c, hipGetLastError());
  }
  if (phaseStats && plan.useFast) {
    unsigned long long h[MM_CW_SKETCH_PHASES_END - MM_CW_SKETCH_PHASES];
    MM_HIP(c, hipMemcpyAsync(h, phaseStats, sizeof h, hipMemcpyDeviceToHost, c->stream));
    MM_HIP(c, hipStreamSynchronize(c->stream));
    fprintf(stderr, "[mm] sketch phases, shader-clock cycles per workgroup (thread 0), %d fragments, %d threads x %d positions, HT %d, queue %d/wave, lds %zu: stage+init %.0f | hash %.0f | wait %.0f | drain %.0f | occupancy+list %.0f | rank+emit %.0f\n",
            nF, g.threads, g.SL, g.HT, g.QC, ldsFast, (double)h[0] / nF, (double)h[1] / nF, (double)h[2] / nF, (double)h[3] / nF, (double)h[4] / nF, (double)h[5] / nF);
  }
  if (c->env.debug) {
    uint32_t nHard = 0;
    MM_HIP(c, hipMemcpyAsync(&nHard, c->dCounters.p, 4, hipMemcpyDeviceToHost, c->stream));
    MM_HIP(c, hipStreamSynchronize(c->stream));
    fprintf(stderr, "[mm] sketch: %d fragments, %u to the hard path%s, threads %d x %d positions, HT %d, lds %zu/%zu%s\n", nF, nHard, plan.useFast ? "" : " (fast kernel not usable at this size)",
            g.threads, g.SL, g.HT, ldsFast, ldsHard, plan.stream ? " (hard table: position / strand arrays in HBM; fragments read from global memory)" : plan.spill ? " (hard table: position / strand arrays in HBM)" : "");
  }
  {
    KernelTimer t(c, MM_K_SKETCH_HARD);
    const int grid = nF < 1024 ? nF : 1024;
    auto launchHard = [&](auto kern, int32_t* spill) {
      (void)hipFuncSetAttribute((const void*)kern, hipFuncAttributeMaxDynamicSharedMemorySize, (int)ldsHard);
      hipLaunchKernelGGL(kern, dim3(grid), dim3(threadsHard), ldsHard, c->stream,
                         c->dSketchTabs.as<uint4>(), c->dBases2.as<uint32_t>(), c->dNmask.as<uint32_t>(), c->dFrags.as<DFrag>(), c->dReadHasN.as<uint32_t>(),
                         c->dHardList.as<int32_t>(), c->dCounters.as<uint32_t>(), s, g.wantFast, HTH, PADH, spill, plan.stream ? 1 : 0, c->dSkHash.as<uint64_t>(), c->dSkPos.as<int2>(), c->dSkStrand.as<int8_t>(),
                         c->dSkCount.as<uint32_t>());
    };
    if (plan.spill) {
      MM_HIP(c, c->dSketchSpill.ensure((size_t)grid * 3 * (size_t)(HTH + PADH) * 4 + 64));
      launchHard(k_sketch_hard<K, true>, c->dSketchSpill.as<int32_t>());
    } else launchHard(k_sketch_hard<K, false>, (int32_t*)nullptr);
    MM_HIP(c, hipGetLastError());
  }
  return MM_OK;
}

template <int K>
static int launch_hash_only_k(mm_ctx* c, int reps, double* msAvg) {
  using Tabs = typename MMTabsFor<K>::type;
  const int nF = (int)c->nFrags;
  const int maxLen = c->maxFragLen;
  const FastGeom g = sketch_fast_geom(K, c->P.sketchSize, maxLen, sizeof(Tabs), MMHasSL20<K>::value);
  const size_t need = sizeof(Tabs) + (((size_t)(maxLen + 15) / 16 + 4) * 4 + 15) / 16 * 16;
  const size_t lds = (g.lds > need && g.lds <= 160 * 1024) ? g.lds : need;
  if (c->sketchTabsK != K) {
    MM_HIP(c, c->dSketchTabs.ensure(sizeof(Tabs)));
    hipLaunchKernelGGL((k_sketch_tables<K>), dim3(1), dim3(256), 0, c->stream, c->dSketchTabs.as<Tabs>());
    MM_HIP(c, hipGetLastError());
    c->sketchTabsK = K;
  }
  MM_HIP(c, c->dCounters.ensure(MM_COUNTER_BYTES));
  float total = 0;
  for (int r = 0; r <= reps; r++) {
    MM_HIP(c, hipEventRecord(c->evA, c->stream));
    auto launch = [&](auto kern) {
      (void)hipFuncSetAttribute((const void*)kern, hipFuncAttributeMaxDynamicSharedMemorySize, (int)lds);
      hipLaunchKernelGGL(kern, dim3(nF), dim3(g.threads), lds, c->stream, c->dSketchTabs.as<uint4>(), c->dBases2.as<uint32_t>(), c->dFrags.as<DFrag>(),
                         c->dCounters.as<uint64_t>() + MM_CW_SKETCH_PHASES);
    };
    if constexpr (MMHasSL20<K>::value) { if (g.SL == 20) launch(k_hash_only<K, 20>); else launch(k_hash_only<K, 16>); }
    else launch(k_hash_only<K, 16>);
    MM_HIP(c, hipGetLastError());
    MM_HIP(c, hipEventRecord(c->evB, c->stream));
    MM_HIP(c, hipEventSynchronize(c->evB));
    float ms = 0; MM_HIP(c, hipEventElapsedTime(&ms, c->evA, c->evB));
    if (r) total += ms;
  }
  *msAvg = total / reps;
  return MM_OK;
}

extern "C" int mm_bench_hash_only(mm_ctx* c, int reps, double* msAvg) {
  if (!c->nFrags || reps < 1 || !msAvg) { c->err = "mm_bench_hash_only: needs resident reads and reps >= 1"; return MM_ERR_ARG; }
  MM_HIP(c, hipSetDevice(c->device));
  switch (c->P.kmerSize) {
#define MM_CASE(KK) case KK: return launch_hash_only_k<KK>(c, reps, msAvg);
    MM_CASE(16) MM_CASE(19) MM_CASE(21)
#undef MM_CASE
    default: c->err = "mm_bench_hash_only: built for k = 16, 19, 21"; return MM_ERR_ARG;
  }
}

int mm_launch_sketch(mm_ctx* c) {
  const size_t nF = c->nFrags, s = (size_t)c->P.sketchSize;
  const size_t cF = mm_frag_cap(c, nF);
  if (s > MM_LDS_MAX_SKETCH) {
    MM_HIP(c, c->dSkHash.ensure(nF * s * 8 + 64)); MM_HIP(c, c->dSkPos.ensure(nF * s * 8 + 64));
    MM_HIP(c, c->dSkStrand.ensure(nF * s + 64)); MM_HIP(c, c->dSkCount.ensure(nF * 4 + 64));
    MM_HIP(c, c->dHardList.ensure(nF * 4 + 64)); MM_HIP(c, c->dCounters.ensure(MM_COUNTER_BYTES));
    MM_HIP(c, hipMemsetAsync(c->dCounters.as<unsigned long long>() + MM_CW_SKETCH, 0, (size_t)(MM_CW_SKETCH_END - MM_CW_SKETCH) * 8, c->stream));
    return mm_launch_sketch_global(c);
  }
  MM_HIP(c, c->dSkHash.ensure(cF * s * 8 + 64));
  MM_HIP(c, c->dSkPos.ensure(cF * s * 8 + 64));
  MM_HIP(c, c->dSkStrand.ensure(cF * s + 64));
  MM_HIP(c, c->dSkCount.ensure(cF * 4 + 64));
  MM_HIP(c, c->dHardList.ensure(cF * 4 + 64));
  MM_HIP(c, c->dCounters.ensure(MM_COUNTER_BYTES));
  if (nF == 0) return MM_OK;
  switch (c->P.kmerSize) {
#define MM_CASE(KK) case KK: return launch_sketch_k<KK>(c);
    MM_CASE(1) MM_CASE(2) MM_CASE(3) MM_CASE(4) MM_CASE(5) MM_CASE(6) MM_CASE(7) MM_CASE(8) MM_CASE(9) MM_CASE(10) MM_CASE(11) MM_CASE(12) MM_CASE(13) MM_CASE(14) MM_CASE(15) MM_CASE(16) MM_CASE(17) MM_CASE(18) MM_CASE(19) MM_CASE(20) MM_CASE(21) MM_CASE(22) MM_CASE(23) MM_CASE(24) MM_CASE(25) MM_CASE(26) MM_CASE(27) MM_CASE(28) MM_CASE(29) MM_CASE(30) MM_CASE(31) MM_CASE(32)
    MM_CASE(33) MM_CASE(34) MM_CASE(35) MM_CASE(36) MM_CASE(37) MM_CASE(38) MM_CASE(39) MM_CASE(40) MM_CASE(41) MM_CASE(42) MM_CASE(43) MM_CASE(44) MM_CASE(45) MM_CASE(46) MM_CASE(47) MM_CASE(48)
    MM_CASE(49) MM_CASE(50) MM_CASE(51) MM_CASE(52) MM_CASE(53) MM_CASE(54) MM_CASE(55) MM_CASE(56) MM_CASE(57) MM_CASE(58) MM_CASE(59) MM_CASE(60) MM_CASE(61) MM_CASE(62) MM_CASE(63) MM_CASE(64)
#undef MM_CASE
    default: c->err = "kmerSize outside 1..64"; return MM_ERR_ARG;
  }
}

int mm_launch_pack_raw(mm_ctx* c, const uint8_t* dAscii, const int64_t* dSrcOff, const int64_t* dPackOff, const int32_t* dLen, int nReads,
                       int64_t nChunks, uint32_t* dB, uint32_t* dM, uint32_t* dHasN) {
  if (nChunks == 0) return MM_OK;
  int blocks = (int)((nChunks + 255) / 256); if (blocks > 16384) blocks = 16384;
  hipLaunchKernelGGL(k_pack2bit, dim3(blocks), dim3(256), 0, c->stream, dAscii, dSrcOff, dPackOff, dLen, nReads, nChunks, dB, dM, dHasN);
  MM_HIP(c, hipGetLastError());
  return MM_OK;
}

int mm_launch_pack(mm_ctx* c) {
  const int64_t nChunks = (int64_t)(c->nPackedBases / 32);
  if (nChunks == 0) return MM_OK;
  KernelTimer t(c, MM_K_PACK);
  int blocks = (int)((nChunks + 255) / 256); if (blocks > 8192) blocks = 8192;
  hipLaunchKernelGGL(k_pack2bit, dim3(blocks), dim3(256), 0, c->stream, c->dAscii.as<uint8_t>(), c->dReadSrcOff.as<int64_t>(),
                     c->dReadPackOff.as<int64_t>(), c->dReadLen.as<int32_t>(), (int)c->nReads, nChunks,
                     c->dBases2.as<uint32_t>(), c->dNmask.as<uint32_t>(), c->dReadHasN.as<uint32_t>());
  MM_HIP(c, hipGetLastError());
  return MM_OK;
}
```

mashmap_amd/csrc/mm_sketch_global.hip:

```cpp
#include "mm_internal.h"
#include "mm_device.h"
#include <algorithm>

namespace {

__device__ __forceinline__ uint32_t g_code(const uint32_t* __restrict__ bases2, int64_t i) { return (bases2[i >> 4] >> (2 * (int)(i & 15))) & 3u; }
__device__ __forceinline__ uint32_t g_ascii(uint32_t code) { return code == 0 ? 0x41u : code == 1 ? 0x43u : code == 2 ? 0x47u : 0x54u; }

__device__ uint64_t g_murmur(const uint32_t* __restrict__ bases2, int64_t b0, int K, bool rc) {
  auto byteAt = [&](int i) -> uint64_t { return rc ? (uint64_t)g_ascii(3u - g_code(bases2, b0 + K - 1 - i)) : (uint64_t)g_ascii(g_code(bases2, b0 + i)); };
  uint64_t h1 = MM_SEED, h2 = MM_SEED;
  const int nb = K / 16;
  for (int b = 0; b < nb; b++) {
    uint64_t k1 = 0, k2 = 0;
    for (int i = 0; i < 8; i++) { k1 |= byteAt(16 * b + i) << (8 * i); k2 |= byteAt(16 * b + 8 + i) << (8 * i); }
    h1 ^= mm_mix_k1(k1); h1 = mm_rotl64(h1, 27); h1 += h2; h1 = h1 * 5 + 0x52dce729;
    h2 ^= mm_mix_k2(k2); h2 = mm_rotl64(h2, 31); h2 += h1; h2 = h2 * 5 + 0x38495ab5;
  }
  const int rem = K & 15;
  uint64_t k1 = 0, k2 = 0;
  for (int i = 0; i < rem; i++) { if (i < 8) k1 |= byteAt(16 * nb + i) << (8 * i); else k2 |= byteAt(16 * nb + i) << (8 * (i - 8)); }
  if (rem > 8) h2 ^= mm_mix_k2(k2);
  if (rem > 0) h1 ^= mm_mix_k1(k1);
  h1 ^= (uint64_t)K; h2 ^= (uint64_t)K;
  h1 += h2; h2 += h1;
  h1 = mm_fmix64(h1); h2 = mm_fmix64(h2);
  return h1 + h2;
}

struct GEnt { uint64_t h; uint32_t m; uint32_t pad; };
__device__ __forceinline__ bool g_less(const GEnt& a, const GEnt& b) { return a.h != b.h ? a.h < b.h : a.m < b.m; }

__global__ void __launch_bounds__(1024)
k_sketch_global(int nF, int K, int s, int64_t slice ,
                const uint32_t* __restrict__ bases2, const uint32_t* __restrict__ nmask, const DFrag* __restrict__ frags, const uint32_t* __restrict__ readHasN,
                GEnt* __restrict__ scratch, uint64_t* __restrict__ skHash, int2* __restrict__ skPos, int8_t* __restrict__ skStrand, uint32_t* __restrict__ skCount) {
  __shared__ int sCount[1024];
  __shared__ int sTotal;
  GEnt* e = scratch + (size_t)blockIdx.x * (size_t)slice;
  const int tid = threadIdx.x, nthr = blockDim.x;
  for (int f = blockIdx.x; f < nF; f += gridDim.x) {
    const DFrag fr = frags[f];
    const int n = fr.len - K + 1;
    if (n <= 0) { if (tid == 0) skCount[f] = 0; continue; }
    const bool hasN = readHasN[fr.readId] != 0;
    const double want = (double)s + 5.0 * sqrt((double)s) + 64.0;
    uint64_t T = want >= (double)n ? MM_HASH_MAX : (uint64_t)(want / (2.0 * (double)n) * 18446744073709551616.0);
    int64_t N2 = 2;
    for (int attempt = 0; attempt < 2; attempt++) {
    if (tid == 0) sTotal = 0;
    __syncthreads();
    for (int64_t p0 = 0; p0 < n; p0 += nthr) {
      const int64_t p = p0 + tid;
      GEnt x; x.h = MM_HASH_MAX; x.m = 0xFFFFFFFFu; x.pad = 0;
      bool keep = false;
      if (p < n) {
        bool ok = true;
        if (hasN) for (int i = 0; i < K && ok; i++) { const int64_t b = fr.base + p + i; if ((nmask[b >> 5] >> (int)(b & 31)) & 1u) ok = false; }
        if (ok) {
          const uint64_t hf = g_murmur(bases2, fr.base + p, K, false), hr = g_murmur(bases2, fr.base + p, K, true);
          if (hf != hr) { x.h = hf < hr ? hf : hr; x.m = ((uint32_t)p << 1) | (hf < hr ? 1u : 0u); keep = T == MM_HASH_MAX || x.h < T; }
        }
      }
      const uint64_t m = mm_ballot(keep);
      int base = 0;
      if (m && mm_lane() == (uint32_t)__builtin_ctzll(m)) base = atomicAdd(&sTotal, (int)__popcll(m));
      if (m) base = __shfl(base, (int)__builtin_ctzll(m));
      if (keep) e[base + (int)mm_popc_below(m)] = x;
    }
    __syncthreads();
    const int nSurv = sTotal;
    N2 = 2; while (N2 < nSurv) N2 <<= 1;
    for (int64_t p = nSurv + tid; p < N2; p += nthr) { GEnt x; x.h = MM_HASH_MAX; x.m = 0xFFFFFFFFu; x.pad = 0; e[p] = x; }
    __threadfence_block();
    __syncthreads();
    for (int64_t k2 = 2; k2 <= N2; k2 <<= 1)
      for (int64_t j = k2 >> 1; j > 0; j >>= 1) {
        for (int64_t i = tid; i < N2; i += nthr) {
          const int64_t q = i ^ j;
          if (q > i) {
            const GEnt a = e[i], b = e[q];
            if (g_less(b, a) == ((i & k2) == 0)) { e[i] = b; e[q] = a; }
          }
        }
        __threadfence_block();
        __syncthreads();
      }
    const int64_t chunk = (N2 + nthr - 1) / nthr;
    const int64_t c0 = (int64_t)tid * chunk, c1 = c0 + chunk < N2 ? c0 + chunk : N2;
    int mine = 0;
    for (int64_t i = c0; i < c1; i++) { const uint64_t h = e[i].h; if (h != MM_HASH_MAX && (i == 0 || e[i - 1].h != h)) mine++; }
    sCount[tid] = mine;
    __syncthreads();
    if (tid == 0) { int acc = 0; for (int t = 0; t < nthr; t++) { const int v = sCount[t]; sCount[t] = acc; acc += v; } sTotal = acc; }
    __syncthreads();
    if (sTotal < s && T != MM_HASH_MAX) { T = MM_HASH_MAX; __syncthreads(); continue; }
    int rank = sCount[tid];
    for (int64_t i = c0; i < c1 && rank < s; i++) {
      const uint64_t h = e[i].h;
      if (h == MM_HASH_MAX || (i != 0 && e[i - 1].h == h)) continue;
      int first = (int)(e[i].m >> 1), last = first, sum = 0;
      for (int64_t r = i; r < N2 && e[r].h == h; r++) { last = (int)(e[r].m >> 1); sum += (e[r].m & 1u) ? 1 : -1; }
      const size_t o = (size_t)f * s + rank;
      skHash[o] = h; skPos[o] = make_int2(first, last);
      const int16_t acc = (int16_t)sum;
      skStrand[o] = acc > 0 ? 1 : (acc == 0 ? 0 : -1);
      rank++;
    }
    if (tid == 0) skCount[f] = (uint32_t)(sTotal < s ? sTotal : s);
    __syncthreads();
    break;
    }
  }
}

}

int mm_launch_sketch_global(mm_ctx* c) {
  const int nF = (int)c->nFrags, K = c->P.kmerSize, s = c->P.sketchSize;
  if (nF == 0) return MM_OK;
  int64_t slice = 2; while (slice < c->maxFragLen) slice <<= 1;
  int grid = (int)std::min<int64_t>(std::min<int64_t>(nF, 1024), std::max<int64_t>(1, ((int64_t)8 << 30) / (slice * (int64_t)sizeof(GEnt))));
  MM_HIP(c, c->dSketchSpill.ensure((size_t)grid * (size_t)slice * sizeof(GEnt) + 64));
  KernelTimer t(c, MM_K_SKETCH_HARD);
  hipLaunchKernelGGL(k_sketch_global, dim3(grid), dim3(1024), 0, c->stream, nF, K, s, slice, c->dBases2.as<uint32_t>(), c->dNmask.as<uint32_t>(), c->dFrags.as<DFrag>(),
                     c->dReadHasN.as<uint32_t>(), c->dSketchSpill.as<GEnt>(), c->dSkHash.as<uint64_t>(), c->dSkPos.as<int2>(), c->dSkStrand.as<int8_t>(),
                     c->dSkCount.as<uint32_t>());
  MM_HIP(c, hipGetLastError());
  return MM_OK;
}
```

Baseline: 164.3.

## Skip sketch position tracking on map path and build occupancy list during insert

```diff
diff --git a/mashmap_amd/csrc/mm_api.hip b/mashmap_amd/csrc/mm_api.hip
--- a/mashmap_amd/csrc/mm_api.hip
+++ b/mashmap_amd/csrc/mm_api.hip
@@ -494,7 +494,7 @@
 
 int mm_sketch_fragments(mm_ctx* c) {
   MM_HIP(c, hipSetDevice(c->device));
-  int rc = mm_launch_sketch(c);
+  int rc = mm_launch_sketch(c, true);
   if (rc != MM_OK) return rc;
   MM_HIP(c, hipStreamSynchronize(c->stream));
   if (c->profile) mm_profile_collect(c);
@@ -505,6 +505,13 @@
 int mm_sketch_download(mm_ctx* c, mm_minmer* out, uint32_t* counts) {
   if (!c->sketched) { c->err = "mm_sketch_download: no sketches resident"; return MM_ERR_STATE; }
   MM_HIP(c, hipSetDevice(c->device));
+  if (!c->skPosValid) {
+    MM_HIP(c, hipStreamSynchronize(c->stream));
+    const bool profile = c->profile; c->profile = false;
+    const int rc = mm_launch_sketch(c, true);
+    c->profile = profile;
+    if (rc != MM_OK) return rc;
+  }
   const size_t nF = c->nFrags, s = (size_t)c->P.sketchSize;
   std::vector<uint64_t> h(nF * s); std::vector<int2> p(nF * s); std::vector<int8_t> st(nF * s); std::vector<uint32_t> cnt(nF);
   if (nF) {
@@ -531,7 +538,7 @@
   MM_HIP(c, hipSetDevice(c->device));
   const auto t0 = std::chrono::steady_clock::now();
   const double a0 = g_mmAllocSeconds;
-  int rc = mm_launch_sketch(c);
+  int rc = mm_launch_sketch(c, false);
   if (rc != MM_OK) return rc;
   c->sketched = true;
   const auto t1 = std::chrono::steady_clock::now();
diff --git a/mashmap_amd/csrc/mm_internal.h b/mashmap_amd/csrc/mm_internal.h
--- a/mashmap_amd/csrc/mm_internal.h
+++ b/mashmap_amd/csrc/mm_internal.h
@@ -227,6 +227,7 @@
   DevBuf dL2InitCells, dL2InitState;
   DevBuf dL2Sort[4], dL2Order, dL2OrderPos;
   bool sketched = false, mapped = false;
+  bool skPosValid = false;
   bool steadyOk = false, lastSteady = false; size_t prevBig = 0, candCap = 0, l2Chunks = 1, sizedFrags = 0; int prevLocap = 0, steadyFails = 0;
   unsigned long long* hPass = nullptr;
   size_t lastHard = 0;
@@ -299,8 +300,8 @@
 int mm_launch_pack(mm_ctx* c);
 int mm_launch_pack_raw(mm_ctx* c, const uint8_t* dAscii, const int64_t* dSrcOff, const int64_t* dPackOff, const int32_t* dLen, int nReads,
                        int64_t nChunks, uint32_t* dB, uint32_t* dM, uint32_t* dHasN);
-int mm_launch_sketch(mm_ctx* c);
-int mm_launch_sketch_global(mm_ctx* c);
+int mm_launch_sketch(mm_ctx* c, bool wantPos);
+int mm_launch_sketch_global(mm_ctx* c, bool wantPos);
 #define MM_LDS_MAX_SKETCH 8190
 #define MM_WINNOW_LDS_SKETCH 4096
 #define MM_MAX_SKETCH 65535
diff --git a/mashmap_amd/csrc/mm_sketch.hip b/mashmap_amd/csrc/mm_sketch.hip
--- a/mashmap_amd/csrc/mm_sketch.hip
+++ b/mashmap_amd/csrc/mm_sketch.hip
@@ -51,7 +51,7 @@
   }
   __device__ __forceinline__ uint32_t home(uint64_t h) const { return __umulhi((uint32_t)((h << sh) >> 32), M); }
 
-  __device__ __forceinline__ void insert(uint64_t h, int pos, int st) {
+  __device__ __forceinline__ void insert(uint64_t h, int pos, int st, const bool wantPos) {
     uint32_t slot = home(h);
     for (uint32_t probes = 1;; probes++) {
       if ((probes & 15u) == 0 && ((volatile uint32_t*)counters)[MM_TC_OVERFLOW]) return;
@@ -61,7 +61,8 @@
         if (atomicAdd(&counters[MM_TC_KEYS], 1u) >= maxLoad) atomicOr(&counters[MM_TC_OVERFLOW], 1u);
       }
       if (prev == MM_HASH_MAX || prev == h) {
-        atomicMin(&first[slot], pos); atomicMax(&last[slot], pos); atomicAdd(&sum[slot], st);
+        if (wantPos) { atomicMin(&first[slot], pos); atomicMax(&last[slot], pos); }
+        atomicAdd(&sum[slot], st);
         return;
       }
       if (++slot >= nSlots) { atomicOr(&counters[MM_TC_OVERFLOW], 1u); return; }
@@ -94,6 +95,7 @@
   if (n <= 0) { if (tid == 0) skCount[f] = 0; return; }
   const bool hasN = readHasN[fr.readId] != 0;
   const uint32_t hint = skCount[f];
+  const bool wantPos = skPos != nullptr;
 
   const int nW = stream ? 0 : (len + 15) / 16 + 3;
   const int nM = stream ? 0 : (len + 31) / 32 + 2;
@@ -183,7 +185,7 @@
         const uint64_t h = hf < hr ? hf : hr;
         bool pass = false;
         if ((ok & (1u << j)) != 0) { if (hf != hr) { if (allPass || h < T) pass = true; } }
-        if (pass) tab.insert(h, pos, hf < hr ? 1 : -1);
+        if (pass) tab.insert(h, pos, hf < hr ? 1 : -1, wantPos);
       };
       if constexpr (MMWideK<K>::value) {
         uint32_t ww[MMWideK<K>::NW];
@@ -249,13 +251,17 @@
     if (rank < (uint32_t)s) {
       const size_t o = (size_t)f * s + rank;
       skHash[o] = k;
-      int vf, vl, vs;
-      if constexpr (SPILL) {
-        vf = __hip_atomic_load(&tab.first[slot], __ATOMIC_RELAXED, __HIP_MEMORY_SCOPE_AGENT);
-        vl = __hip_atomic_load(&tab.last[slot], __ATOMIC_RELAXED, __HIP_MEMORY_SCOPE_AGENT);
-        vs = __hip_atomic_load(&tab.sum[slot], __ATOMIC_RELAXED, __HIP_MEMORY_SCOPE_AGENT);
-      } else { vf = tab.first[slot]; vl = tab.last[slot]; vs = tab.sum[slot]; }
-      skPos[o] = make_int2(vf, vl);
+      int vs;
+      if constexpr (SPILL) vs = __hip_atomic_load(&tab.sum[slot], __ATOMIC_RELAXED, __HIP_MEMORY_SCOPE_AGENT);
+      else vs = tab.sum[slot];
+      if (wantPos) {
+        int vf, vl;
+        if constexpr (SPILL) {
+          vf = __hip_atomic_load(&tab.first[slot], __ATOMIC_RELAXED, __HIP_MEMORY_SCOPE_AGENT);
+          vl = __hip_atomic_load(&tab.last[slot], __ATOMIC_RELAXED, __HIP_MEMORY_SCOPE_AGENT);
+        } else { vf = tab.first[slot]; vl = tab.last[slot]; }
+        skPos[o] = make_int2(vf, vl);
+      }
       const int16_t acc = (int16_t)vs;
       skStrand[o] = acc > 0 ? 1 : (acc == 0 ? 0 : -1);
     }
@@ -288,7 +294,7 @@
 struct SkFast {
   uint64_t* key; uint32_t* meta;
   uint32_t* dup; uint32_t* counters;
-  uint64_t* occW; uint32_t* occP;
+  uint64_t* occW;
   uint32_t nSlots, maxLoad, M; int sh;
   __device__ __forceinline__ void set_cut(uint64_t T, uint32_t HT) {
     sh = (T == MM_HASH_MAX) ? 0 : __clzll((long long)T);
@@ -300,7 +306,11 @@
     uint32_t slot = home(h);
     for (;;) {
       const unsigned long long prev = atomicCAS((unsigned long long*)&key[slot], (unsigned long long)MM_HASH_MAX, (unsigned long long)h);
-      if (prev == MM_HASH_MAX) { meta[slot] = m; return; }
+      if (prev == MM_HASH_MAX) {
+        meta[slot] = m;
+        atomicOr(&((uint32_t*)occW)[slot >> 5], 1u << (slot & 31u));
+        return;
+      }
       if (prev == h) {
         const uint32_t at = atomicAdd(&counters[MM_TC_DUPS], 1u);
         if (at < MM_SK_DUPCAP) dup[at] = slot | (m << 13); else atomicOr(&counters[MM_TC_OVERFLOW], 1u);
@@ -311,7 +321,7 @@
   }
 };
 
-template <int K, int SL>
+template <int K, int SL, bool WANT_POS>
 __device__ __forceinline__ void
 mm_sketch_fast(unsigned char* smem, const int f, const uint4* __restrict__ gTabs, const uint32_t* __restrict__ bases2, const uint32_t* __restrict__ nmask,
                const DFrag* __restrict__ frags, const uint32_t* __restrict__ readHasN, int s, int wantFast, int HT, int PAD, int QC,
@@ -347,7 +357,7 @@
   tab.key = (uint64_t*)(smem + off) + MM_SK_GUARD; off += (size_t)(NS + 2 * MM_SK_GUARD) * 8;
   tab.occW = (uint64_t*)(smem + off); off += (size_t)nOcc * 8;
   tab.meta = (uint32_t*)(smem + off); off += (size_t)NS * 4;
-  tab.occP = (uint32_t*)(smem + off); off += (((size_t)nOcc * 4 + 15) / 16) * 16;
+  off += (((size_t)nOcc * 4 + 15) / 16) * 16;
   uint32_t* qCnt = (uint32_t*)(smem + off); off += 64;
   tab.dup = (uint32_t*)(smem + off); off += (size_t)MM_SK_DUPCAP * 4;
   tab.counters = (uint32_t*)(smem + off); off += 16;
@@ -371,6 +381,7 @@
   const int nStrips = (n + SL - 1) / SL;
   tab.set_cut(T, (uint32_t)HT);
   for (int i = tid; i < NS; i += nthr) tab.key[i] = MM_HASH_MAX;
+  for (int i = tid; i < nOcc; i += nthr) tab.occW[i] = 0ull;
   if (tid < MM_SK_GUARD) { tab.key[-1 - tid] = MM_HASH_MAX; tab.key[NS + tid] = MM_HASH_MAX; }
   if (tid < 4) tab.counters[tid] = 0;
   __syncthreads();
@@ -432,12 +443,22 @@
     for (int w = 0; w < 16; w++) pre[w + 1] = pre[w] + (w < nWaves ? qCnt[w] : 0u);
     const uint32_t total = pre[16];
     if (nWaves <= 4) {
-      const uint32_t p1 = pre[1], p2 = pre[2], p3 = pre[3];
-      for (uint32_t g = (uint32_t)tid; g < total; g += (uint32_t)nthr) {
-        const uint32_t w = (g >= p1 ? 1u : 0u) + (g >= p2 ? 1u : 0u) + (g >= p3 ? 1u : 0u);
-        const uint32_t start = g >= p3 ? p3 : (g >= p2 ? p2 : (g >= p1 ? p1 : 0u));
-        const uint32_t at = w * (uint32_t)QC + (g - start);
-        tab.insert(qH[at], qM[at]);
+      auto rfl = [](uint32_t x) { return (uint32_t)__builtin_amdgcn_readfirstlane((int)x); };
+      const uint32_t p1 = rfl(pre[1]), p2 = rfl(pre[2]), p3 = rfl(pre[3]), p4 = rfl(total);
+      auto place = [&](uint32_t g, uint32_t& w, uint32_t& start) {
+        w = (g >= p1 ? 1u : 0u) + (g >= p2 ? 1u : 0u) + (g >= p3 ? 1u : 0u);
+        start = g >= p3 ? p3 : (g >= p2 ? p2 : (g >= p1 ? p1 : 0u));
+      };
+      for (uint32_t g0 = rfl((uint32_t)tid & ~63u); g0 < p4; g0 += (uint32_t)nthr) {
+        const uint32_t gl = g0 + 63u < p4 ? g0 + 63u : p4 - 1u;
+        uint32_t wA, startA, wL, startL;
+        place(g0, wA, startA); place(gl, wL, startL);
+        const uint32_t endA = wA == 0 ? p1 : (wA == 1 ? p2 : (wA == 2 ? p3 : p4));
+        const uint32_t g = g0 + mm_lane();
+        uint32_t at;
+        if (wL == wA || endA == startL) at = g + (g >= startL ? wL * (uint32_t)QC - startL : wA * (uint32_t)QC - startA);
+        else { uint32_t w, start; place(g, w, start); at = w * (uint32_t)QC + (g - start); }
+        if (g < p4) tab.insert(qH[at], qM[at]);
       }
     } else
     for (uint32_t g = (uint32_t)tid; g < total; g += (uint32_t)nthr) {
@@ -454,35 +475,30 @@
     const uint32_t nd = tab.counters[MM_TC_DUPS] < MM_SK_DUPCAP ? tab.counters[MM_TC_DUPS] : MM_SK_DUPCAP;
     for (uint32_t i = (uint32_t)tid; i < nd; i += (uint32_t)nthr) atomicOr(&tab.meta[tab.dup[i] & 0x1FFFu], MM_SKF_FLAG);
   }
-  for (int base = 0; base < NS; base += nthr) {
-    const int slot = base + tid;
-    if (slot < NS) {
-      const uint64_t m = __ballot(tab.key[slot] != MM_HASH_MAX);
-      if (mm_lane() == 0) tab.occW[slot >> 6] = m;
-    }
-  }
-  __syncthreads();
-  if (tid < 64) {
-    int carry = 0;
+  uint32_t* occList = qM;
+  uint32_t D = 0;
+  {
+    const int wave = __builtin_amdgcn_readfirstlane(tid >> 6);
+    const int lane = (int)mm_lane();
+    int mine = wave;
     for (int w0 = 0; w0 < nOcc; w0 += 64) {
-      const int w = w0 + tid;
-      const int v = w < nOcc ? (int)__popcll(tab.occW[w]) : 0;
+      const int nw = nOcc - w0 < 64 ? nOcc - w0 : 64;
+      const uint64_t mw = lane < nw ? tab.occW[w0 + lane] : 0ull;
+      const int v = (int)__popcll(mw);
       const int ex = mm_wave_excl_scan(v);
-      if (w < nOcc) tab.occP[w] = (uint32_t)(carry + ex);
-      carry += mm_wave_sum(v);
-    }
-    if (tid == 0) { tab.counters[MM_TC_OCCUPIED] = (uint32_t)carry; if ((uint32_t)carry > tab.maxLoad) tab.counters[MM_TC_OVERFLOW] = 1u; }
-  }
-  __syncthreads();
-  const uint32_t D = tab.counters[MM_TC_OCCUPIED];
-  if (tab.counters[MM_TC_OVERFLOW] != 0 || (D < (uint32_t)s && T != MM_HASH_MAX)) {
-    if (tid == 0) { const uint32_t at = atomicAdd(hardCount, 1u); hardList[at] = f; skCount[f] = tab.counters[MM_TC_OVERFLOW] != 0 ? MM_SK_HINT_OVERFLOW : D; }
+      for (; mine < w0 + nw; mine += nWaves) {
+        const int x = mine - w0;
+        const uint64_t m = (uint64_t)(uint32_t)__builtin_amdgcn_readlane((int)(uint32_t)mw, x) | ((uint64_t)(uint32_t)__builtin_amdgcn_readlane((int)(uint32_t)(mw >> 32), x) << 32);
+        const uint32_t before = D + (uint32_t)__builtin_amdgcn_readlane(ex, x);
+        if (__builtin_amdgcn_inverse_ballot_w64(m)) occList[before + mm_popc_below(m)] = (uint32_t)(mine * 64 + lane);
+      }
+      D += (uint32_t)mm_wave_sum(v);
+    }
+  }
+  const bool overflow = tab.counters[MM_TC_OVERFLOW] != 0 || D > tab.maxLoad;
+  if (overflow || (D < (uint32_t)s && T != MM_HASH_MAX)) {
+    if (tid == 0) { const uint32_t at = atomicAdd(hardCount, 1u); hardList[at] = f; skCount[f] = overflow ? MM_SK_HINT_OVERFLOW : D; }
     return;
-  }
-  uint32_t* occList = qM;
-  for (int slot = tid; slot < NS; slot += nthr) {
-    const uint64_t m = tab.occW[slot >> 6];
-    if ((m >> (slot & 63)) & 1ull) occList[tab.occP[slot >> 6] + (uint32_t)__popcll(m & ((1ull << (slot & 63)) - 1ull))] = (uint32_t)slot;
   }
   __syncthreads();
   mark(4);
@@ -514,13 +530,13 @@
         for (uint32_t i = 0; i < nDup; i++) {
           const uint32_t d = tab.dup[i];
           if ((int)(d & 0x1FFFu) != slot) continue;
-          const int pos = (int)(d >> 14);
-          first = pos < first ? pos : first; last = pos > last ? pos : last; sum += ((d >> 13) & 1u) ? 1 : -1;
+          if constexpr (WANT_POS) { const int pos = (int)(d >> 14); first = pos < first ? pos : first; last = pos > last ? pos : last; }
+          sum += ((d >> 13) & 1u) ? 1 : -1;
         }
       }
       const size_t o = (size_t)f * s + rank;
       skHash[o] = k;
-      skPos[o] = make_int2(first, last);
+      if constexpr (WANT_POS) skPos[o] = make_int2(first, last);
       const int16_t acc = (int16_t)sum;
       skStrand[o] = acc > 0 ? 1 : (acc == 0 ? 0 : -1);
     }
@@ -529,7 +545,7 @@
   mark(5);
 }
 
-template <int K, int SL>
+template <int K, int SL, bool WANT_POS>
 __global__ void __launch_bounds__(1024)
 k_sketch_fast(const uint4* __restrict__ gTabs, const uint32_t* __restrict__ bases2, const uint32_t* __restrict__ nmask,
               const DFrag* __restrict__ frags, const uint32_t* __restrict__ readHasN, int s, int wantFast, int HT, int PAD, int QC,
@@ -537,7 +553,7 @@
               uint32_t* __restrict__ skCount, int32_t* __restrict__ hardList, uint32_t* __restrict__ hardCount,
               unsigned long long* __restrict__ phaseStats) {
   extern __shared__ __attribute__((aligned(16))) unsigned char smem[];
-  mm_sketch_fast<K, SL>(smem, (int)blockIdx.x, gTabs, bases2, nmask, frags, readHasN, s, wantFast, HT, PAD, QC, skHash, skPos, skStrand, skCount,
+  mm_sketch_fast<K, SL, WANT_POS>(smem, (int)blockIdx.x, gTabs, bases2, nmask, frags, readHasN, s, wantFast, HT, PAD, QC, skHash, skPos, skStrand, skCount,
                         hardList, hardCount, phaseStats);
 }
 
@@ -687,7 +703,7 @@
 template <int K> struct MMHasSL20 { static constexpr bool value = (K >= 16 && K <= 21); };
 
 template <int K>
-static int launch_sketch_k(mm_ctx* c) {
+static int launch_sketch_k(mm_ctx* c, const bool wantPos) {
   const int s = c->P.sketchSize;
   const int nF = (int)c->nFrags;
   using Tabs = typename MMTabsFor<K>::type;
@@ -715,11 +731,14 @@
       (void)hipFuncSetAttribute((const void*)kern, hipFuncAttributeMaxDynamicSharedMemorySize, (int)ldsFast);
       hipLaunchKernelGGL(kern, dim3(nF), dim3(g.threads), ldsFast, c->stream,
                          c->dSketchTabs.as<uint4>(), c->dBases2.as<uint32_t>(), c->dNmask.as<uint32_t>(), c->dFrags.as<DFrag>(), c->dReadHasN.as<uint32_t>(),
-                         s, g.wantFast, g.HT, PAD, g.QC, c->dSkHash.as<uint64_t>(), c->dSkPos.as<int2>(), c->dSkStrand.as<int8_t>(),
+                         s, g.wantFast, g.HT, PAD, g.QC, c->dSkHash.as<uint64_t>(), wantPos ? c->dSkPos.as<int2>() : (int2*)nullptr, c->dSkStrand.as<int8_t>(),
                          c->dSkCount.as<uint32_t>(), c->dHardList.as<int32_t>(), c->dCounters.as<uint32_t>(), phaseStats);
     };
-    if constexpr (MMHasSL20<K>::value) { if (g.SL == 20) launch(k_sketch_fast<K, 20>); else launch(k_sketch_fast<K, 16>); }
-    else launch(k_sketch_fast<K, 16>);
+    auto launchSL = [&](auto sl) {
+      if (wantPos) launch(k_sketch_fast<K, decltype(sl)::value, true>); else launch(k_sketch_fast<K, decltype(sl)::value, false>);
+    };
+    if constexpr (MMHasSL20<K>::value) { if (g.SL == 20) launchSL(std::integral_constant<int, 20>{}); else launchSL(std::integral_constant<int, 16>{}); }
+    else launchSL(std::integral_constant<int, 16>{});
     MM_HIP(c, hipGetLastError());
   } else {
     KernelTimer t(c, MM_K_SKETCH);
@@ -747,7 +766,7 @@
       (void)hipFuncSetAttribute((const void*)kern, hipFuncAttributeMaxDynamicSharedMemorySize, (int)ldsHard);
       hipLaunchKernelGGL(kern, dim3(grid), dim3(threadsHard), ldsHard, c->stream,
                          c->dSketchTabs.as<uint4>(), c->dBases2.as<uint32_t>(), c->dNmask.as<uint32_t>(), c->dFrags.as<DFrag>(), c->dReadHasN.as<uint32_t>(),
-                         c->dHardList.as<int32_t>(), c->dCounters.as<uint32_t>(), s, g.wantFast, HTH, PADH, spill, plan.stream ? 1 : 0, c->dSkHash.as<uint64_t>(), c->dSkPos.as<int2>(), c->dSkStrand.as<int8_t>(),
+                         c->dHardList.as<int32_t>(), c->dCounters.as<uint32_t>(), s, g.wantFast, HTH, PADH, spill, plan.stream ? 1 : 0, c->dSkHash.as<uint64_t>(), wantPos ? c->dSkPos.as<int2>() : (int2*)nullptr, c->dSkStrand.as<int8_t>(),
                          c->dSkCount.as<uint32_t>());
     };
     if (plan.spill) {
@@ -805,31 +824,37 @@
   }
 }
 
-int mm_launch_sketch(mm_ctx* c) {
+int mm_launch_sketch(mm_ctx* c, bool wantPos) {
   const size_t nF = c->nFrags, s = (size_t)c->P.sketchSize;
+  c->skPosValid = false;
   const size_t cF = mm_frag_cap(c, nF);
   if (s > MM_LDS_MAX_SKETCH) {
-    MM_HIP(c, c->dSkHash.ensure(nF * s * 8 + 64)); MM_HIP(c, c->dSkPos.ensure(nF * s * 8 + 64));
+    MM_HIP(c, c->dSkHash.ensure(nF * s * 8 + 64)); if (wantPos) MM_HIP(c, c->dSkPos.ensure(nF * s * 8 + 64));
     MM_HIP(c, c->dSkStrand.ensure(nF * s + 64)); MM_HIP(c, c->dSkCount.ensure(nF * 4 + 64));
     MM_HIP(c, c->dHardList.ensure(nF * 4 + 64)); MM_HIP(c, c->dCounters.ensure(MM_COUNTER_BYTES));
     MM_HIP(c, hipMemsetAsync(c->dCounters.as<unsigned long long>() + MM_CW_SKETCH, 0, (size_t)(MM_CW_SKETCH_END - MM_CW_SKETCH) * 8, c->stream));
-    return mm_launch_sketch_global(c);
+    const int rc = mm_launch_sketch_global(c, wantPos);
+    if (rc == MM_OK) c->skPosValid = wantPos;
+    return rc;
   }
   MM_HIP(c, c->dSkHash.ensure(cF * s * 8 + 64));
-  MM_HIP(c, c->dSkPos.ensure(cF * s * 8 + 64));
+  if (wantPos) MM_HIP(c, c->dSkPos.ensure(cF * s * 8 + 64));
   MM_HIP(c, c->dSkStrand.ensure(cF * s + 64));
   MM_HIP(c, c->dSkCount.ensure(cF * 4 + 64));
   MM_HIP(c, c->dHardList.ensure(cF * 4 + 64));
   MM_HIP(c, c->dCounters.ensure(MM_COUNTER_BYTES));
-  if (nF == 0) return MM_OK;
+  if (nF == 0) { c->skPosValid = wantPos; return MM_OK; }
+  int rc = MM_ERR_ARG;
   switch (c->P.kmerSize) {
-#define MM_CASE(KK) case KK: return launch_sketch_k<KK>(c);
+#define MM_CASE(KK) case KK: rc = launch_sketch_k<KK>(c, wantPos); break;
     MM_CASE(1) MM_CASE(2) MM_CASE(3) MM_CASE(4) MM_CASE(5) MM_CASE(6) MM_CASE(7) MM_CASE(8) MM_CASE(9) MM_CASE(10) MM_CASE(11) MM_CASE(12) MM_CASE(13) MM_CASE(14) MM_CASE(15) MM_CASE(16) MM_CASE(17) MM_CASE(18) MM_CASE(19) MM_CASE(20) MM_CASE(21) MM_CASE(22) MM_CASE(23) MM_CASE(24) MM_CASE(25) MM_CASE(26) MM_CASE(27) MM_CASE(28) MM_CASE(29) MM_CASE(30) MM_CASE(31) MM_CASE(32)
     MM_CASE(33) MM_CASE(34) MM_CASE(35) MM_CASE(36) MM_CASE(37) MM_CASE(38) MM_CASE(39) MM_CASE(40) MM_CASE(41) MM_CASE(42) MM_CASE(43) MM_CASE(44) MM_CASE(45) MM_CASE(46) MM_CASE(47) MM_CASE(48)
     MM_CASE(49) MM_CASE(50) MM_CASE(51) MM_CASE(52) MM_CASE(53) MM_CASE(54) MM_CASE(55) MM_CASE(56) MM_CASE(57) MM_CASE(58) MM_CASE(59) MM_CASE(60) MM_CASE(61) MM_CASE(62) MM_CASE(63) MM_CASE(64)
 #undef MM_CASE
     default: c->err = "kmerSize outside 1..64"; return MM_ERR_ARG;
   }
+  if (rc == MM_OK) c->skPosValid = wantPos;
+  return rc;
 }
 
 int mm_launch_pack_raw(mm_ctx* c, const uint8_t* dAscii, const int64_t* dSrcOff, const int64_t* dPackOff, const int32_t* dLen, int nReads,
diff --git a/mashmap_amd/csrc/mm_sketch_global.hip b/mashmap_amd/csrc/mm_sketch_global.hip
--- a/mashmap_amd/csrc/mm_sketch_global.hip
+++ b/mashmap_amd/csrc/mm_sketch_global.hip
@@ -102,7 +102,7 @@
       int first = (int)(e[i].m >> 1), last = first, sum = 0;
       for (int64_t r = i; r < N2 && e[r].h == h; r++) { last = (int)(e[r].m >> 1); sum += (e[r].m & 1u) ? 1 : -1; }
       const size_t o = (size_t)f * s + rank;
-      skHash[o] = h; skPos[o] = make_int2(first, last);
+      skHash[o] = h; if (skPos) skPos[o] = make_int2(first, last);
       const int16_t acc = (int16_t)sum;
       skStrand[o] = acc > 0 ? 1 : (acc == 0 ? 0 : -1);
       rank++;
@@ -116,7 +116,7 @@
 
 }
 
-int mm_launch_sketch_global(mm_ctx* c) {
+int mm_launch_sketch_global(mm_ctx* c, bool wantPos) {
   const int nF = (int)c->nFrags, K = c->P.kmerSize, s = c->P.sketchSize;
   if (nF == 0) return MM_OK;
   int64_t slice = 2; while (slice < c->maxFragLen) slice <<= 1;
@@ -124,7 +124,7 @@
   MM_HIP(c, c->dSketchSpill.ensure((size_t)grid * (size_t)slice * sizeof(GEnt) + 64));
   KernelTimer t(c, MM_K_SKETCH_HARD);
   hipLaunchKernelGGL(k_sketch_global, dim3(grid), dim3(1024), 0, c->stream, nF, K, s, slice, c->dBases2.as<uint32_t>(), c->dNmask.as<uint32_t>(), c->dFrags.as<DFrag>(),
-                     c->dReadHasN.as<uint32_t>(), c->dSketchSpill.as<GEnt>(), c->dSkHash.as<uint64_t>(), c->dSkPos.as<int2>(), c->dSkStrand.as<int8_t>(),
+                     c->dReadHasN.as<uint32_t>(), c->dSketchSpill.as<GEnt>(), c->dSkHash.as<uint64_t>(), wantPos ? c->dSkPos.as<int2>() : (int2*)nullptr, c->dSkStrand.as<int8_t>(),
                      c->dSkCount.as<uint32_t>());
   MM_HIP(c, hipGetLastError());
   return MM_OK;
```

New measurement: 164.2. No clear change (-0.1%).
